# PABannier/bark.cpp

Measured on NVIDIA H100. Metric: audio sec/sec (inverse RTF), bark-small f16, batch 1 per GPU, semantic->coarse->fine->encodec, higher is better.
Workload: dtype f16 weights/operands, f32 accumulate (reference arithmetic)

## Files before the change

### bark.cpp_b200/__init__.py

```python
from __future__ import annotations

import ctypes as C
import os

import numpy as np

_HERE = os.path.dirname(os.path.abspath(__file__))
LIB_PATH = os.path.join(_HERE, "libbark_b200.so")

PROGRESS_CB = C.CFUNCTYPE(None, C.c_void_p, C.c_int, C.c_int, C.c_void_p)


class BarkContextParams(C.Structure):
    _fields_ = [
        ("verbosity", C.c_int), ("temp", C.c_float), ("fine_temp", C.c_float), ("min_eos_p", C.c_float),
        ("sliding_window_size", C.c_int32), ("max_coarse_history", C.c_int32), ("sample_rate", C.c_int32),
        ("target_bandwidth", C.c_int32), ("cls_token_id", C.c_int32), ("sep_token_id", C.c_int32),
        ("n_steps_text_encoder", C.c_int32), ("text_pad_token", C.c_int32), ("text_encoding_offset", C.c_int32),
        ("semantic_rate_hz", C.c_float), ("semantic_pad_token", C.c_int32), ("semantic_vocab_size", C.c_int32),
        ("semantic_infer_token", C.c_int32), ("coarse_rate_hz", C.c_float), ("coarse_infer_token", C.c_int32),
        ("coarse_semantic_pad_token", C.c_int32), ("n_coarse_codebooks", C.c_int32), ("n_fine_codebooks", C.c_int32),
        ("codebook_size", C.c_int32), ("progress_callback", PROGRESS_CB), ("progress_callback_user_data", C.c_void_p),
    ]


class BarkStatistics(C.Structure):
    _fields_ = [("t_load_us", C.c_int64), ("t_eval_us", C.c_int64), ("t_semantic_us", C.c_int64), ("t_coarse_us", C.c_int64),
                ("t_fine_us", C.c_int64), ("n_sample_semantic", C.c_int32), ("n_sample_coarse", C.c_int32), ("n_sample_fine", C.c_int32)]


EXPORTS = [
    "bark_context_default_params", "bark_load_model", "bark_generate_audio", "bark_get_audio_data", "bark_get_audio_data_size",
    "bark_get_load_time", "bark_get_eval_time", "bark_reset_statistics", "bark_model_quantize", "bark_free",
    "bark_b200_set_device", "bark_b200_version", "bark_b200_gpt_eval", "bark_b200_fine_eval", "bark_b200_encodec_decode",
    "bark_b200_sample", "bark_b200_sample_rows", "bark_b200_reseed", "bark_b200_tokenize", "bark_b200_forward_text_encoder",
    "bark_b200_forward_coarse_encoder", "bark_b200_forward_fine_encoder", "bark_b200_get_tokens", "bark_b200_set_tokens",
    "bark_b200_get_stats", "bark_b200_get_hparams", "bark_b200_kernel_launches", "bark_b200_layernorm_fallbacks",
    "bark_b200_profile_enable", "bark_b200_profile_report", "bark_b200_io_counters", "bark_b200_decode_timing",
    "bark_b200_shard_init", "bark_b200_shard_connect", "bark_b200_shard_nvlink_bytes",
    "bark_b200_fast_mode", "bark_b200_fast_gemm", "bark_b200_fast_attention",
    "bark_b200_generate_batch", "bark_b200_batch_audio", "bark_b200_batch_tokens", "bark_b200_gpt_eval_slot", "bark_b200_gpt_step_batch",
    "ggml_time_init", "ggml_time_us", "ggml_time_ms", "ggml_init", "ggml_free",
]

_lib = None


def lib() -> C.CDLL:
    global _lib
    if _lib is not None:
        return _lib
    if not os.path.exists(LIB_PATH):
        raise RuntimeError(f"{LIB_PATH} is missing: build the CUDA extension first (python -c 'import __graft_entry__ as g; g.build()'). "
                           "There is no CPU fallback.")
    L = C.CDLL(LIB_PATH)
    vp, i32p, f32p = C.c_void_p, C.c_void_p, C.c_void_p
    L.bark_context_default_params.restype = BarkContextParams
    L.bark_load_model.restype = vp
    L.bark_load_model.argtypes = [C.c_char_p, BarkContextParams, C.c_uint32]
    L.bark_generate_audio.restype = C.c_bool
    L.bark_generate_audio.argtypes = [vp, C.c_char_p, C.c_int]
    L.bark_get_audio_data.restype = C.POINTER(C.c_float)
    L.bark_get_audio_data.argtypes = [vp]
    L.bark_get_audio_data_size.restype = C.c_int
    L.bark_get_audio_data_size.argtypes = [vp]
    for n in ("bark_get_load_time", "bark_get_eval_time"):
        getattr(L, n).restype = C.c_int64
        getattr(L, n).argtypes = [vp]
    L.bark_reset_statistics.argtypes = [vp]
    L.bark_model_quantize.restype = C.c_bool
    L.bark_model_quantize.argtypes = [C.c_char_p, C.c_char_p, C.c_int]
    L.bark_free.argtypes = [vp]
    L.bark_b200_set_device.argtypes = [C.c_int]
    L.bark_b200_version.restype = C.c_char_p
    L.bark_b200_gpt_eval.restype = C.c_int
    L.bark_b200_gpt_eval.argtypes = [vp, C.c_int, i32p, C.c_int, C.POINTER(C.c_int), C.c_int, f32p]
    L.bark_b200_fine_eval.restype = C.c_int
    L.bark_b200_fine_eval.argtypes = [vp, i32p, C.c_int, f32p]
    L.bark_b200_encodec_decode.restype = C.c_int
    L.bark_b200_encodec_decode.argtypes = [vp, i32p, C.c_int, f32p, C.c_int]
    L.bark_b200_sample.restype = C.c_int
    L.bark_b200_sample.argtypes = [vp, C.c_int, f32p, C.c_int, C.c_float, C.POINTER(C.c_float)]
    L.bark_b200_sample_rows.restype = C.c_int
    L.bark_b200_sample_rows.argtypes = [vp, f32p, C.c_int, C.c_int, C.c_float, i32p, f32p]
    L.bark_b200_reseed.argtypes = [vp, C.c_uint32]
    L.bark_b200_tokenize.argtypes = [vp, C.c_char_p, i32p]
    for n in ("bark_b200_forward_text_encoder", "bark_b200_forward_coarse_encoder", "bark_b200_forward_fine_encoder"):
        getattr(L, n).restype = C.c_bool
        getattr(L, n).argtypes = [vp, C.c_int]
    L.bark_b200_get_tokens.restype = C.c_int
    L.bark_b200_get_tokens.argtypes = [vp, C.c_int, i32p, C.c_int]
    L.bark_b200_set_tokens.argtypes = [vp, C.c_int, i32p, C.c_int]
    L.bark_b200_get_stats.argtypes = [vp, C.POINTER(BarkStatistics), C.c_void_p]
    L.bark_b200_get_hparams.argtypes = [vp, C.c_int, i32p]
    L.bark_b200_kernel_launches.restype = C.c_ulonglong
    L.bark_b200_layernorm_fallbacks.restype = C.c_uint
    L.bark_b200_layernorm_fallbacks.argtypes = [vp]
    L.bark_b200_profile_enable.argtypes = [C.c_int]
    L.bark_b200_profile_report.restype = C.c_int
    L.bark_b200_profile_report.argtypes = [C.c_char_p, C.c_int]
    L.bark_b200_io_counters.argtypes = [C.POINTER(C.c_ulonglong), C.POINTER(C.c_ulonglong), C.c_int]
    L.bark_b200_decode_timing.restype = C.c_int
    L.bark_b200_decode_timing.argtypes = [vp, C.c_void_p, C.c_int]
    L.bark_b200_shard_init.restype = C.c_int
    L.bark_b200_shard_init.argtypes = [vp, C.c_int, C.c_int, vp]
    L.bark_b200_shard_connect.restype = C.c_int
    L.bark_b200_shard_connect.argtypes = [vp, vp]
    L.bark_b200_shard_nvlink_bytes.restype = C.c_ulonglong
    L.bark_b200_shard_nvlink_bytes.argtypes = [vp, C.c_int]
    L.bark_b200_fast_mode.restype = C.c_int
    L.bark_b200_fast_mode.argtypes = [vp]
    L.bark_b200_fast_gemm.restype = C.c_int
    L.bark_b200_fast_gemm.argtypes = [vp, vp, vp, C.c_int, C.c_int, C.c_int, C.c_int, C.c_int]
    L.bark_b200_fast_attention.restype = C.c_int
    L.bark_b200_fast_attention.argtypes = [vp, vp, vp, vp, C.c_int, C.c_int, C.c_int]
    L.bark_b200_generate_batch.restype = C.c_bool
    L.bark_b200_generate_batch.argtypes = [vp, C.POINTER(C.c_char_p), C.POINTER(C.c_uint32), C.c_int, C.c_int]
    L.bark_b200_batch_audio.restype = C.c_int
    L.bark_b200_batch_audio.argtypes = [vp, C.c_int, f32p, C.c_int]
    L.bark_b200_batch_tokens.restype = C.c_int
    L.bark_b200_batch_tokens.argtypes = [vp, C.c_int, C.c_int, i32p, C.c_int]
    L.bark_b200_gpt_eval_slot.restype = C.c_int
    L.bark_b200_gpt_eval_slot.argtypes = [vp, C.c_int, C.c_int, i32p, C.c_int, C.POINTER(C.c_int), C.c_int, f32p]
    L.bark_b200_gpt_step_batch.restype = C.c_int
    L.bark_b200_gpt_step_batch.argtypes = [vp, C.c_int, C.c_int, i32p, i32p, i32p, f32p]
    L.ggml_time_us.restype = C.c_int64
    _lib = L
    return L


def _p(a: np.ndarray):
    return a.ctypes.data_as(C.c_void_p)


class Bark:

    def __init__(self, model_path: str, seed: int = 0, n_steps_text_encoder: int | None = None, temp=None, fine_temp=None,
                 min_eos_p=None, device: int | None = None, progress=None):
        L = lib()
        p = L.bark_context_default_params()
        if n_steps_text_encoder is not None:
            p.n_steps_text_encoder = n_steps_text_encoder
        if temp is not None:
            p.temp = temp
        if fine_temp is not None:
            p.fine_temp = fine_temp
        if min_eos_p is not None:
            p.min_eos_p = min_eos_p
        self._cb = PROGRESS_CB(progress) if progress else PROGRESS_CB()
        p.progress_callback = self._cb
        if device is not None:
            L.bark_b200_set_device(device)
        self.params = p
        self.ctx = L.bark_load_model(os.fsencode(model_path), p, seed)
        if not self.ctx:
            raise RuntimeError(f"bark_load_model failed for {model_path} (see stderr); no CPU fallback exists")
        self.ctx = C.c_void_p(self.ctx)

    def close(self):
        if getattr(self, "ctx", None):
            lib().bark_free(self.ctx)
            self.ctx = None

    def __enter__(self):
        return self

    def __exit__(self, *a):
        self.close()

    def generate(self, text: str, n_threads: int = 1) -> np.ndarray:
        if not lib().bark_generate_audio(self.ctx, text.encode(), n_threads):
            raise RuntimeError("bark_generate_audio failed")
        n = lib().bark_get_audio_data_size(self.ctx)
        return np.ctypeslib.as_array(lib().bark_get_audio_data(self.ctx), shape=(n,)).copy()

    @property
    def load_time_us(self):
        return lib().bark_get_load_time(self.ctx)

    @property
    def eval_time_us(self):
        return lib().bark_get_eval_time(self.ctx)

    def hparams(self, which: int) -> np.ndarray:
        a = np.zeros(10, np.int32)
        lib().bark_b200_get_hparams(self.ctx, which, _p(a))
        return a

    def tokens(self, stage: int) -> np.ndarray:
        n = lib().bark_b200_get_tokens(self.ctx, stage, None, 0)
        a = np.zeros(max(n, 1), np.int32)
        lib().bark_b200_get_tokens(self.ctx, stage, _p(a), n)
        a = a[:n]
        return a.reshape(-1, 2) if stage == 1 else a.reshape(-1, 8) if stage == 2 else a

    def set_tokens(self, stage: int, arr):
        a = np.ascontiguousarray(arr, np.int32).ravel()
        lib().bark_b200_set_tokens(self.ctx, stage, _p(a), a.size)

    def tokenize(self, text: str) -> np.ndarray:
        a = np.zeros(513, np.int32)
        lib().bark_b200_tokenize(self.ctx, text.encode(), _p(a))
        return a

    def gpt_eval(self, which: int, tokens, n_past: int, merge_ctx: bool):
        t = np.ascontiguousarray(tokens, np.int32)
        out = np.zeros(int(self.hparams(which)[6]), np.float32)
        np_ = C.c_int(n_past)
        if not lib().bark_b200_gpt_eval(self.ctx, which, _p(t), t.size, C.byref(np_), int(merge_ctx), _p(out)):
            raise RuntimeError("bark_b200_gpt_eval failed")
        return out, np_.value

    def gpt_eval_slot(self, which: int, slot: int, tokens, n_past: int, merge_ctx: bool):
        t = np.ascontiguousarray(tokens, np.int32)
        out = np.zeros(int(self.hparams(which)[6]), np.float32)
        np_ = C.c_int(n_past)
        if not lib().bark_b200_gpt_eval_slot(self.ctx, which, slot, _p(t), t.size, C.byref(np_), int(merge_ctx), _p(out)):
            raise RuntimeError("bark_b200_gpt_eval_slot failed")
        return out, np_.value

    def gpt_step_batch(self, which: int, slots, tokens, n_past):
        sl = np.ascontiguousarray(slots, np.int32); t = np.ascontiguousarray(tokens, np.int32)
        npa = np.array(n_past, np.int32, copy=True)
        assert sl.size == t.size == npa.size
        out = np.zeros((sl.size, int(self.hparams(which)[6])), np.float32)
        if not lib().bark_b200_gpt_step_batch(self.ctx, which, sl.size, _p(sl), _p(t), _p(npa), _p(out)):
            raise RuntimeError("bark_b200_gpt_step_batch failed")
        return out, npa

    def generate_batch(self, texts, seeds, n_threads: int = 1) -> list:
        n = len(texts)
        if len(seeds) != n:
            raise RuntimeError(f"generate_batch: {n} prompts but {len(seeds)} seeds")
        arr = (C.c_char_p * max(n, 1))(*[t.encode() for t in texts])
        sd = (C.c_uint32 * max(n, 1))(*[int(s) for s in seeds])
        if not lib().bark_b200_generate_batch(self.ctx, arr, sd, n, n_threads):
            raise RuntimeError("bark_b200_generate_batch failed")
        out = []
        for i in range(n):
            m = lib().bark_b200_batch_audio(self.ctx, i, None, 0)
            a = np.zeros(max(m, 1), np.float32)
            lib().bark_b200_batch_audio(self.ctx, i, _p(a), m)
            out.append(a[:m])
        return out

    def batch_tokens(self, i: int, stage: int) -> np.ndarray:
        n = lib().bark_b200_batch_tokens(self.ctx, i, stage, None, 0)
        if n < 0:
            raise IndexError(f"no batch item {i}")
        a = np.zeros(max(n, 1), np.int32)
        lib().bark_b200_batch_tokens(self.ctx, i, stage, _p(a), n)
        a = a[:n]
        return a.reshape(-1, 2) if stage == 1 else a.reshape(-1, 8) if stage == 2 else a

    def fine_eval(self, in_buffer, nn: int) -> np.ndarray:
        t = np.ascontiguousarray(in_buffer, np.int32)
        assert t.size == 8 * 1024
        out = np.zeros((1024, int(self.hparams(2)[6])), np.float32)
        if not lib().bark_b200_fine_eval(self.ctx, _p(t), nn, _p(out)):
            raise RuntimeError("bark_b200_fine_eval failed")
        return out

    def encodec_decode(self, codes_8xT) -> np.ndarray:
        c = np.ascontiguousarray(codes_8xT, np.int32)
        T = c.shape[1]
        out = np.zeros(320 * T, np.float32)
        n = lib().bark_b200_encodec_decode(self.ctx, _p(c), T, _p(out), out.size)
        if n < 0:
            raise RuntimeError("bark_b200_encodec_decode failed")
        return out[:n]

    def sample(self, which: int, logits, temp: float):
        l = np.ascontiguousarray(logits, np.float32)
        e = C.c_float(0)
        return lib().bark_b200_sample(self.ctx, which, _p(l), l.size, temp, C.byref(e)), e.value

    def sample_rows(self, logits_rows, temp: float):
        l = np.ascontiguousarray(logits_rows, np.float32)
        rows, n = l.shape
        tok = np.zeros(rows, np.int32); eos = np.zeros(rows, np.float32)
        r = lib().bark_b200_sample_rows(self.ctx, _p(l), n, rows, temp, _p(tok), _p(eos))
        if r < 0:
            raise RuntimeError("bark_b200_sample_rows failed")
        return tok, eos, r

    def reseed(self, seed: int):
        lib().bark_b200_reseed(self.ctx, seed)

    def forward(self, stage: int):
        f = [lib().bark_b200_forward_text_encoder, lib().bark_b200_forward_coarse_encoder, lib().bark_b200_forward_fine_encoder][stage]
        if not f(self.ctx, 1):
            raise RuntimeError("stage failed")

    def stats(self):
        s = BarkStatistics()
        pm = np.zeros(9, np.int64)
        lib().bark_b200_get_stats(self.ctx, C.byref(s), _p(pm))
        return s, pm.reshape(3, 3)

    def shard_init(self, rank: int, world: int) -> bytes:
        h = C.create_string_buffer(64)
        if not lib().bark_b200_shard_init(self.ctx, rank, world, C.cast(h, C.c_void_p)):
            raise RuntimeError("bark_b200_shard_init failed")
        return h.raw

    def shard_connect(self, all_handles: bytes):
        buf = C.create_string_buffer(all_handles, len(all_handles))
        if not lib().bark_b200_shard_connect(self.ctx, C.cast(buf, C.c_void_p)):
            raise RuntimeError("bark_b200_shard_connect failed")

    def shard_nvlink_bytes(self, reset: bool = False) -> int:
        return int(lib().bark_b200_shard_nvlink_bytes(self.ctx, int(reset)))

    @property
    def fast_mode(self) -> bool:
        return bool(lib().bark_b200_fast_mode(self.ctx))

    def layernorm_fallbacks(self) -> int:
        return int(lib().bark_b200_layernorm_fallbacks(self.ctx))


FAST_EPILOGUES = {"f32": 0, "resid": 1, "gelu16": 2, "qkv16": 4}


class GuardBandError(RuntimeError):
    """The GEMM stored outside its output."""


def fast_gemm(A: np.ndarray, W: np.ndarray, epilogue: str = "f32", bn: int = 0, resid: np.ndarray | None = None, return_bn: bool = False):
    A = np.ascontiguousarray(A, np.float16); W = np.ascontiguousarray(W, np.float16)
    M, K = A.shape; N = W.shape[0]
    assert W.shape[1] == K, (A.shape, W.shape)
    if epilogue == "resid":
        out = np.array(resid, np.float32, order="C", copy=True)
        assert out.shape == (M, N), out.shape
    elif epilogue == "qkv16":
        assert N % 6 == 0, N
        out = np.zeros(M * N, np.float16)
    else:
        out = np.zeros((M, N), np.float16 if epilogue == "gelu16" else np.float32)
    r = lib().bark_b200_fast_gemm(_p(A), _p(W), _p(out), M, N, K, FAST_EPILOGUES[epilogue], bn)
    if r == -1:
        raise GuardBandError(f"bark_b200_fast_gemm ({epilogue}, {M}x{N}x{K}, bn {bn}) wrote outside its output")
    if r <= 0:
        raise RuntimeError(f"bark_b200_fast_gemm ({epilogue}, {M}x{N}x{K}, bn {bn}) failed")
    if epilogue == "qkv16":
        out = (out[:M * 2 * N // 3].reshape(M, 2 * N // 3), out[M * 2 * N // 3:].reshape(N // 3, M))
    return (out, r) if return_bn else out


def fast_attention(q: np.ndarray, k: np.ndarray, v: np.ndarray, n_head: int) -> np.ndarray:
    q, k, v = (np.ascontiguousarray(a, np.float16) for a in (q, k, v))
    n, E = q.shape
    out = np.zeros((n, E), np.float16)
    if not lib().bark_b200_fast_attention(_p(q), _p(k), _p(v), _p(out), n, E, n_head):
        raise RuntimeError("bark_b200_fast_attention failed")
    return out


def kernel_launches() -> int:
    return int(lib().bark_b200_kernel_launches())


def profile_enable(on: bool):
    lib().bark_b200_profile_enable(int(on))


def profile_report() -> dict:
    import json
    n = lib().bark_b200_profile_report(None, 0)
    buf = C.create_string_buffer(n + 16)
    lib().bark_b200_profile_report(buf, n + 16)
    return json.loads(buf.value.decode())


def io_counters(reset: bool = False):
    a, b = C.c_ulonglong(0), C.c_ulonglong(0)
    lib().bark_b200_io_counters(C.byref(a), C.byref(b), int(reset))
    return a.value, b.value
```

### bark.cpp_b200/csrc/bark_api.cu

```cuda
#include "../../include/bark_b200.h"
#include "context.h"
#include "gpt_kernels.h"

#include <algorithm>
#include <cmath>
#include <cstring>

using namespace bark;

namespace {

thread_local int g_device_override = -1;
bool quiet() { static const bool q = [] { const char * e = getenv("BARK_B200_QUIET"); return e && *e && *e != '0'; }(); return q; }

inline bool is_alpha(unsigned char c) { return (c >= 'a' && c <= 'z') || (c >= 'A' && c <= 'Z'); }
inline bool is_digit(unsigned char c) { return c >= '0' && c <= '9'; }
inline bool is_punct(unsigned char c) { return c > 32 && c < 127 && !is_alpha(c) && !is_digit(c); }

char fold_accent(unsigned char second) {
    const unsigned cp = 0xC0u + (second - 0x80u);
    const bool lower = cp >= 0xE0;
    const unsigned up = lower ? cp - 0x20 : cp;
    char base = 0;
    if (up >= 0xC0 && up <= 0xC5) base = 'A';
    else if (up == 0xC7) base = 'C';
    else if (up >= 0xC8 && up <= 0xCB) base = 'E';
    else if (up >= 0xCC && up <= 0xCF) base = 'I';
    else if (up == 0xD1) base = 'N';
    else if (up >= 0xD2 && up <= 0xD6) base = 'O';
    else if (up >= 0xD9 && up <= 0xDC) base = 'U';
    else if (up == 0xDD) base = 'Y';
    if (!base) return 0;
    return lower ? (char)(base + 32) : base;
}

std::string strip_accents_utf8(const std::string & in) {
    std::string out;
    for (size_t i = 0; i < in.size();) {
        const unsigned char c = (unsigned char) in[i];
        const unsigned hi = c >> 4;
        size_t len = hi < 12 ? 1 : hi < 14 ? 2 : hi == 14 ? 3 : 4;
        len = std::min(len, in.size() - i);
        char folded = 0;
        if (len == 2 && c == 0xC3) { const unsigned char d = (unsigned char) in[i + 1]; if (d >= 0x80 && d <= 0xBF) folded = fold_accent(d); }
        if (folded) out.push_back(folded); else out.append(in, i, len);
        i += len;
    }
    return out;
}

void wordpiece(const std::map<std::string, int32_t> & vocab, const std::string & text, std::vector<int32_t> & out, int n_max_tokens) {
    const std::string s = strip_accents_utf8(text);
    out.clear();
    size_t i = 0;
    while (i < s.size()) {
        const unsigned char c = (unsigned char) s[i];
        size_t j = i;
        if (is_punct(c)) j = i + 1;
        else if (is_alpha(c)) { while (j < s.size() && is_alpha((unsigned char) s[j])) j++; }
        else if (is_digit(c)) { while (j < s.size() && is_digit((unsigned char) s[j])) j++; }
        else { i++; continue; }
        const std::string word = s.substr(i, j - i);
        i = j;
        size_t p = 0; bool cont = false;
        while (p < word.size()) {
            if ((int) out.size() >= n_max_tokens - 1) break;
            size_t e = word.size(); bool hit = false;
            for (; e > p; e--) {
                auto it = vocab.find((cont ? "##" : "") + word.substr(p, e - p));
                if (it != vocab.end()) { out.push_back(it->second); p = e; cont = true; hit = true; break; }
            }
            if (!hit) { fprintf(stderr, "%s: unknown token '%c'\n", "bert_tokenize", word[p]); cont = true; p++; }
        }
    }
}

void tokenize_input(bark_context * ctx, Generation & g, const std::string & text) {
    const bark_context_params & P = ctx->params;
    const int max_ctx = std::min(ctx->semantic.block_size, 256);
    std::vector<int32_t> pieces;
    wordpiece(ctx->token_to_id, text, pieces, max_ctx);
    std::vector<int32_t> t((size_t) max_ctx, 0);
    std::copy(pieces.begin(), pieces.end(), t.begin());
    for (auto & v : t) v += P.text_encoding_offset;
    for (size_t k = pieces.size(); k < t.size(); k++) t[k] = P.text_pad_token;
    t.insert(t.end(), 256, P.semantic_pad_token);
    t.push_back(P.semantic_infer_token);
    g.tokens = t;
    if (!quiet()) {
        printf("%s: prompt: '%s'\n", "bark_tokenize_input", text.c_str());
        printf("%s: number of tokens in prompt = %zu, first 8 tokens: ", "bark_tokenize_input", g.tokens.size());
        for (size_t k = 0; k < std::min<size_t>(8, g.tokens.size()); k++) printf("%d ", g.tokens[k]);
        printf("\n\n");
    }
}

int32_t sample_token(std::mt19937 & rng, GPTModel & m, const float * logits, int n, float temp, float * eos_p) {
    const int64_t t0 = now_us();
    std::vector<float> p(logits, logits + n);
    const float div = temp == 0.0f ? 0.7f : temp;
    for (float & v : p) v /= div;
    float mx = -INFINITY;
    for (float v : p) mx = std::max(mx, v);
    float sum = 0.0f;
    for (float & v : p) { v = (float) exp((double)(v - mx)); sum += v; }
    for (float & v : p) v /= sum;
    int32_t next = 0;
    if (temp == 0.0f) {
        float best = -INFINITY;
        for (int i = 0; i < n; i++) if (p[(size_t) i] > best) { best = p[(size_t) i]; next = i; }
    } else {
        std::discrete_distribution<int32_t> dist(p.begin(), p.end());
        next = dist(rng);
    }
    if (eos_p) *eos_p = p.back();
    m.t_sample_us += now_us() - t0;
    m.n_sample += 1;
    return next;
}

}

int32_t bark::sample_token_given_u(const float * logits, int n, float temp, double u, float * eos_p) {
    std::vector<float> p(logits, logits + n);
    const float div = temp == 0.0f ? 0.7f : temp;
    for (float & v : p) v /= div;
    float mx = -INFINITY;
    for (float v : p) mx = std::max(mx, v);
    float sum = 0.0f;
    for (float & v : p) { v = (float) exp((double)(v - mx)); sum += v; }
    for (float & v : p) v /= sum;
    if (eos_p) *eos_p = p.back();
    if (temp == 0.0f) {
        float best = -INFINITY; int32_t next = 0;
        for (int i = 0; i < n; i++) if (p[(size_t) i] > best) { best = p[(size_t) i]; next = i; }
        return next;
    }
    std::vector<double> cp(p.begin(), p.end());
    double tot = 0.0;
    for (double v : cp) tot += v;
    for (double & v : cp) v /= tot;
    for (size_t i = 1; i < cp.size(); i++) cp[i] += cp[i - 1];
    cp.back() = 1.0;
    return (int32_t)(std::lower_bound(cp.begin(), cp.end(), u) - cp.begin());
}

namespace {

void print_stage_stats(const GPTModel & m) {
    if (quiet()) return;
    printf("\n\n");
    printf("%s:   sample time = %8.2f ms / %lld tokens\n", "bark_print_statistics", m.t_sample_us / 1000.0f, (long long) m.n_sample);
    printf("%s:  predict time = %8.2f ms / %.2f ms per token\n", "bark_print_statistics", m.t_predict_us / 1000.0f,
           m.n_sample ? m.t_predict_us / (double) m.n_sample / 1000.0 : 0.0);
    printf("%s:    total time = %8.2f ms\n", "bark_print_statistics", m.t_main_us / 1000.0f);
    printf("\n");
}

template <typename LoOf>
bool run_chain(bark_context * ctx, std::mt19937 & rng, GPTModel & m, const std::vector<int32_t> & first_in, bool merge_ctx, int * n_past, int n, LoOf lo_of, int samp_n, float temp,
               int32_t * out_tok, float * out_eos) {
    if (n < 1 || n > 1024) return false;
    const int64_t t_begin = now_us();
    cudaStream_t s = ctx->stream;
    if (temp != 0.0f) {
        for (int j = 0; j < n; j++) ctx->h_u[j] = std::generate_canonical<double, 53>(rng);
        BARK_CUDA_CHECK(cudaMemcpyAsync(ctx->d_u, ctx->h_u, (size_t) n * sizeof(double), cudaMemcpyHostToDevice, s)); bark::g_h2d_bytes += (size_t) n * sizeof(double);
    }
    const bool chain = ctx->use_decode_kernel && m.decode_ok;
    std::vector<int> past_before((size_t) n);
    std::vector<int32_t> cur_in = first_in;
    std::vector<float> host_logits;
    int start = 0;
    while (start < n) {
        const int stop = chain ? n : start + 1;
        for (int j = start; j < stop; j++) {
            const int lo = lo_of(j);
            past_before[(size_t) j] = *n_past;
            if (j == start) { if (!gpt_eval(ctx, m, cur_in.data(), (int) cur_in.size(), n_past, merge_ctx && *n_past == 0, nullptr, lo, lo + samp_n)) return false; }
            const int force = ctx->debug_flag_every > 0 && (ctx->n_sample_calls++ % ctx->debug_flag_every) == 0;
            if (j > start && !gpt_decode_chained(ctx, m, ctx->d_feed, n_past, lo, lo + samp_n)) return false;
            sample_rows(ctx->last_logits + lo, m.n_out_vocab, samp_n, 1, temp, ctx->d_u + j, ctx->d_stok + j, lo, ctx->d_feed, ctx->d_seos + j, ctx->d_sflags + j, force, s);
        }
        const size_t cnt = (size_t)(stop - start);
        BARK_CUDA_CHECK(cudaMemcpyAsync(ctx->h_stok + start, ctx->d_stok + start, cnt * 4, cudaMemcpyDeviceToHost, s));
        BARK_CUDA_CHECK(cudaMemcpyAsync(ctx->h_sflags + start, ctx->d_sflags + start, cnt * 4, cudaMemcpyDeviceToHost, s));
        BARK_CUDA_CHECK(cudaMemcpyAsync(ctx->h_seos + start, ctx->d_seos + start, cnt * 4, cudaMemcpyDeviceToHost, s)); bark::g_d2h_bytes += cnt * 12;
        BARK_CUDA_CHECK(cudaStreamSynchronize(s));
        int f = start;
        while (f < stop && !ctx->h_sflags[f]) f++;
        if (f == stop) { start = stop; if (start < n) cur_in.assign(1, ctx->h_stok[start - 1]); continue; }
        if (f > start) cur_in.assign(1, ctx->h_stok[f - 1]);
        *n_past = past_before[(size_t) f];
        const int lo = lo_of(f);
        host_logits.resize((size_t) m.n_out_vocab);
        if (!gpt_eval(ctx, m, cur_in.data(), (int) cur_in.size(), n_past, merge_ctx && *n_past == 0, host_logits.data(), lo, lo + samp_n)) return false;
        ctx->h_stok[f] = lo + sample_token_given_u(host_logits.data() + lo, samp_n, temp, ctx->h_u[f], &ctx->h_seos[f]);
        ctx->n_sample_host_replays++;
        start = f + 1;
        cur_in.assign(1, ctx->h_stok[f]);
    }
    for (int j = 0; j < n; j++) { out_tok[j] = ctx->h_stok[j]; if (out_eos) out_eos[j] = ctx->h_seos[j]; }
    m.n_sample += n;
    m.t_predict_us += now_us() - t_begin;
    return true;
}

bool run_semantic(bark_context * ctx, Generation & g) {
    const int64_t t_start = now_us();
    GPTModel & m = ctx->semantic;
    const bark_context_params & P = ctx->params;
    std::vector<float> logits((size_t) m.n_out_vocab);
    std::vector<int32_t> input = g.tokens, output;
    int n_past = 0; float eos_p = 0.0f;
    const bool dev = ctx->sample_on_device && (size_t) m.n_out_vocab * 4 <= 64 * 1024;
    if (dev) {
        constexpr int kBatch = 64;
        std::vector<int32_t> tok(kBatch); std::vector<float> eos(kBatch);
        bool done = false;
        for (int i = 0; i < P.n_steps_text_encoder && !done; i += kBatch) {
            const int nb = std::min(kBatch, P.n_steps_text_encoder - i);
            const std::mt19937 saved = g.rng;
            if (!run_chain(ctx, g.rng, m, input, true, &n_past, nb, [](int) { return 0; }, m.n_out_vocab, P.temp, tok.data(), eos.data())) { fprintf(stderr, "%s: Could not generate token\n", __func__); return false; }
            for (int j = 0; j < nb; j++) {
                if (P.progress_callback) P.progress_callback(ctx, SEMANTIC, 100 * (i + j + 1) / P.n_steps_text_encoder, P.progress_callback_user_data);
                if (tok[(size_t) j] == P.semantic_vocab_size || eos[(size_t) j] >= P.min_eos_p) {
                    if (P.temp != 0.0f) { g.rng = saved; for (int k = 0; k <= j; k++) (void) std::generate_canonical<double, 53>(g.rng); }
                    m.n_sample -= nb - (j + 1);
                    done = true; break;
                }
                output.push_back(tok[(size_t) j]);
            }
            if (!done && nb > 0) input.assign(1, tok[(size_t) nb - 1]);
        }
    } else
    for (int i = 0; i < P.n_steps_text_encoder; i++) {
        if (P.progress_callback) P.progress_callback(ctx, SEMANTIC, 100 * (i + 1) / P.n_steps_text_encoder, P.progress_callback_user_data);
        if (!gpt_eval(ctx, m, input.data(), (int) input.size(), &n_past, true, logits.data())) { fprintf(stderr, "%s: Could not generate token\n", __func__); return false; }
        const int32_t next = sample_token(g.rng, m, logits.data(), m.n_out_vocab, P.temp, &eos_p);
        if (next == P.semantic_vocab_size || eos_p >= P.min_eos_p) break;
        input.assign(1, next);
        output.push_back(next);
    }
    g.semantic_tokens = output;
    ctx->stats.n_sample_semantic = (int32_t) m.n_sample;
    m.t_main_us = now_us() - t_start;
    ctx->stats.t_semantic_us = m.t_main_us;
    print_stage_stats(m);
    return true;
}

int coarse_n_steps(const bark_context_params & P, size_t n_semantic) {
    const float stc_ratio = P.coarse_rate_hz / P.semantic_rate_hz * P.n_coarse_codebooks;
    return (int)(floorf(n_semantic * stc_ratio / P.n_coarse_codebooks) * P.n_coarse_codebooks);
}

std::vector<int32_t> coarse_window(bark_context * ctx, const std::vector<int32_t> & sem, const std::vector<int32_t> & out, int step,
                                   std::vector<int32_t> & kv_ids, size_t & kv_canon, int * n_past) {
    const bark_context_params & P = ctx->params;
    const float stc_ratio = P.coarse_rate_hz / P.semantic_rate_hz * P.n_coarse_codebooks;
    const int max_semantic_history = (int) floorf(P.max_coarse_history / stc_ratio);
    const int semantic_idx = (int) roundf(step / stc_ratio);
    std::vector<int32_t> in(sem.begin() + std::max(semantic_idx - max_semantic_history, 0), sem.end());
    in.resize(256, P.coarse_semantic_pad_token);
    in.push_back(P.coarse_infer_token);
    const size_t hist = std::min<size_t>((size_t) P.max_coarse_history, out.size());
    in.insert(in.end(), out.end() - (std::ptrdiff_t) hist, out.end());
    *n_past = 0;
    if (ctx->kv_reuse) {
        size_t common = 0;
        while (common < kv_ids.size() && common < in.size() && kv_ids[common] == in[common]) common++;
        *n_past = (int) std::min({common, kv_canon, in.size() & ~(size_t) 31, in.size() - 1});
        ctx->n_kv_reused += (unsigned long long) *n_past;
    }
    kv_canon = std::max((size_t) *n_past, in.size() & ~(size_t) 31);
    std::vector<int32_t> in_eval(in.begin() + *n_past, in.end());
    kv_ids = in;
    return in_eval;
}

void store_coarse_tokens(const bark_context_params & P, const std::vector<int32_t> & out, std::vector<int32_t> & coarse) {
    coarse.resize(out.size());
    for (size_t i = 0; i + 1 < out.size(); i += 2) {
        coarse[i] = out[i] - P.semantic_vocab_size;
        coarse[i + 1] = out[i + 1] - P.semantic_vocab_size - P.codebook_size;
    }
}

bool run_coarse(bark_context * ctx, Generation & g) {
    const int64_t t_start = now_us();
    GPTModel & m = ctx->coarse;
    const bark_context_params & P = ctx->params;
    const std::vector<int32_t> & sem = g.semantic_tokens;
    std::vector<float> logits((size_t) m.n_out_vocab);
    const int n_steps = coarse_n_steps(P, sem.size());
    if (n_steps <= 0 || P.n_coarse_codebooks != 2) { fprintf(stderr, "%s: nothing to generate (%zu semantic tokens)\n", __func__, sem.size()); return false; }
    const int n_windows = (int) ceilf((float) n_steps / P.sliding_window_size);
    std::vector<int32_t> out; out.reserve((size_t) n_steps);
    const bool dev = ctx->sample_on_device && P.sliding_window_size <= 1024 && P.semantic_vocab_size + 2 * P.codebook_size <= m.n_out_vocab;
    int step = 0;
    std::vector<int32_t> kv_ids;
    size_t kv_canon = 0;
    for (int w = 0; w < n_windows; w++) {
        int n_past = 0;
        std::vector<int32_t> in_eval = coarse_window(ctx, sem, out, step, kv_ids, kv_canon, &n_past);
        if (dev) {
            const int nw = std::min(P.sliding_window_size, n_steps - step), step0 = step;
            std::vector<int32_t> tok((size_t) nw);
            auto lo_of = [&](int j) { return P.semantic_vocab_size + (((step0 + j) % P.n_coarse_codebooks == 0) ? 0 : 1) * P.codebook_size; };
            if (!run_chain(ctx, g.rng, m, in_eval, false, &n_past, nw, lo_of, P.codebook_size, P.temp, tok.data(), nullptr)) { fprintf(stderr, "%s: Could not generate token\n", __func__); return false; }
            for (int j = 0; j < nw; j++) {
                if (P.progress_callback) P.progress_callback(ctx, COARSE, 100 * (step + 1) / n_steps, P.progress_callback_user_data);
                out.push_back(tok[(size_t) j]); step++;
                if (j + 1 < nw) kv_ids.push_back(tok[(size_t) j]);
            }
            continue;
        }
        for (int j = 0; j < P.sliding_window_size && step < n_steps; j++) {
            if (P.progress_callback) P.progress_callback(ctx, COARSE, 100 * (step + 1) / n_steps, P.progress_callback_user_data);
            const bool major = step % P.n_coarse_codebooks == 0;
            const int lo = P.semantic_vocab_size + (major ? 0 : 1) * P.codebook_size;
            if (j > 0) kv_ids.push_back(in_eval[0]);
            if (!gpt_eval(ctx, m, in_eval.data(), (int) in_eval.size(), &n_past, false, logits.data(), lo, lo + P.codebook_size)) { fprintf(stderr, "%s: Could not generate token\n", __func__); return false; }
            const int32_t next = lo + sample_token(g.rng, m, logits.data() + lo, P.codebook_size, P.temp, nullptr);
            in_eval.assign(1, next);
            out.push_back(next);
            step++;
        }
    }
    store_coarse_tokens(P, out, g.coarse_tokens);
    ctx->stats.n_sample_coarse = (int32_t) m.n_sample;
    m.t_main_us = now_us() - t_start;
    ctx->stats.t_coarse_us = m.t_main_us;
    print_stage_stats(m);
    return true;
}

bool run_fine(bark_context * ctx, Generation & g, bool progress = true) {
    const int64_t t_start = now_us();
    GPTModel & m = ctx->fine;
    const bark_context_params & P = ctx->params;
    const int n_coarse = P.n_coarse_codebooks, n_cb = P.n_fine_codebooks, cb_size = P.codebook_size;
    if (n_cb != 8 || n_coarse != 2 || cb_size != 1024) { fprintf(stderr, "%s: unsupported codebook configuration\n", __func__); return false; }
    const int T = (int) g.coarse_tokens.size() / 2;
    const int len = std::max(T, 1024);
    std::vector<int32_t> arr((size_t) len * 8, cb_size);
    for (int t = 0; t < T; t++) { arr[(size_t) t * 8] = g.coarse_tokens[(size_t) t * 2]; arr[(size_t) t * 8 + 1] = g.coarse_tokens[(size_t) t * 2 + 1]; }
    const int n_loops = std::max(0, (int) ceilf((len - 1024) / 512.f)) + 1;
    std::vector<float> logits((size_t) 1024 * m.n_out_vocab);
    std::vector<int32_t> buf((size_t) 8 * 1024), sampled(1024);
    const bool dev = ctx->sample_on_device;
    for (int n = 0; n < n_loops; n++) {
        const int start = std::min(n * 512, len - 1024), fill = std::min(n * 512, len - 512), rel = fill - start;
        for (int c = 0; c < 8; c++) for (int j = 0; j < 1024; j++) buf[(size_t) c * 1024 + j] = arr[(size_t)(start + j) * 8 + c];
        for (int nn = n_coarse; nn < n_cb; nn++) {
            if (progress && P.progress_callback) P.progress_callback(ctx, FINE, 100 * (n * (n_cb - n_coarse) + (nn - n_coarse + 1)) / (n_loops * (n_cb - n_coarse)), P.progress_callback_user_data);
            if (ctx->shard.on) {
                if (!fine_eval_shard(ctx, buf.data(), nn) || !sample_shard(ctx, g.rng, cb_size, P.fine_temp, sampled.data())) { fprintf(stderr, "%s: Could not generate token\n", __func__); return false; }
            } else {
            if (!fine_eval(ctx, buf.data(), nn, dev ? nullptr : logits.data())) { fprintf(stderr, "%s: Could not generate token\n", __func__); return false; }
            if (dev && !sample_device(ctx, m, g.rng, ctx->last_logits, m.n_out_vocab, cb_size, 1024, P.fine_temp, sampled.data(), nullptr)) return false;
            }
            for (int i = 0; i < 1024; i++) {
                const int32_t next = (dev || ctx->shard.on) ? sampled[(size_t) i] : sample_token(g.rng, m, logits.data() + (size_t) i * m.n_out_vocab, cb_size, P.fine_temp, nullptr);
                if (i >= rel) buf[(size_t) nn * 1024 + i] = next;
            }
        }
        for (int nn = n_coarse; nn < n_cb; nn++) for (int j = 0; j < 1024 - rel; j++) arr[(size_t)(fill + j) * 8 + nn] = buf[(size_t) nn * 1024 + rel + j];
    }
    g.fine_tokens.assign(arr.begin(), arr.begin() + (std::ptrdiff_t) T * 8);
    ctx->stats.n_sample_fine = (int32_t) m.n_sample;
    m.t_main_us = now_us() - t_start;
    ctx->stats.t_fine_us = m.t_main_us;
    print_stage_stats(m);
    return true;
}

bool decode_audio(bark_context * ctx, Generation & g) {
    const int T = (int) g.fine_tokens.size() / 8;
    std::vector<int32_t> codes((size_t) 8 * T);
    for (int c = 0; c < 8; c++) for (int t = 0; t < T; t++) codes[(size_t) c * T + t] = g.fine_tokens[(size_t) t * 8 + c];
    if (ctx->params.target_bandwidth != 6 || ctx->params.sample_rate != 24000) {
        fprintf(stderr, "%s: only target_bandwidth 6 / 24 kHz is implemented\n", __func__); return false;
    }
    if (!codec_decode(ctx, codes.data(), T, g.audio)) { printf("%s: Could not generate waveform from tokens with Encodec\n", __func__); return false; }
    return true;
}

constexpr int kMaxBatch = 8;

bool ensure_batch_slots(bark_context * ctx, int n) {
    BatchSlots & S = ctx->batch;
    auto fail = [&](const char * what) { (void) cudaGetLastError(); fprintf(stderr, "bark_b200: out of device memory for %s\n", what); return false; };
    if (!S.d_logits) {
        const size_t n_out = (size_t) std::max(ctx->semantic.n_out_vocab, ctx->coarse.n_out_vocab);
        float * l = nullptr; int32_t * d = nullptr, * h = nullptr;
        if (cudaMalloc(&l, kMaxBatch * n_out * 4) != cudaSuccess) return fail("the batch logits");
        if (cudaMalloc(&d, 16 * 4) != cudaSuccess) { cudaFree(l); return fail("the batch logits"); }
        if (cudaMallocHost(&h, 16 * 4) != cudaSuccess) { cudaFree(l); cudaFree(d); return fail("the batch logits"); }
        S.d_logits = l; S.d_step = d; S.h_step = h;
    }
    for (; S.cap < n; S.cap++) {
        float * slab[4] = {nullptr, nullptr, nullptr, nullptr};
        size_t bytes[4];
        for (int j = 0; j < 4; j++) {
            const GPTModel & m = j < 2 ? ctx->semantic : ctx->coarse;
            bytes[j] = (size_t) m.n_layer * m.block_size * m.n_embd * 4;
            if (cudaMalloc(&slab[j], bytes[j]) != cudaSuccess) {
                for (int q = 0; q < j; q++) cudaFree(slab[q]);
                return fail("a batch item's KV cache");
            }
        }
        for (int j = 0; j < 4; j++) BARK_CUDA_CHECK(cudaMemsetAsync(slab[j], 0, bytes[j], ctx->stream));
        S.k[0][S.cap] = slab[0]; S.v[0][S.cap] = slab[1]; S.k[1][S.cap] = slab[2]; S.v[1][S.cap] = slab[3];
    }
    return true;
}

struct BatchItem {
    Generation g;
    int n_past = 0;
    std::vector<int32_t> out, kv_ids;
    size_t kv_canon = 0;
    int n_steps = 0;
};

bool batch_prefill(bark_context * ctx, GPTModel & m, int which, BatchItem & it, int b, int row, const std::vector<int32_t> & in, bool merge, int lo, int hi) {
    BatchSlots & S = ctx->batch;
    if (!gpt_eval(ctx, m, in.data(), (int) in.size(), &it.n_past, merge, nullptr, lo, hi, S.k[which][b], S.v[which][b])) return false;
    BARK_CUDA_CHECK(cudaMemcpyAsync(S.d_logits + (size_t) row * m.n_out_vocab, ctx->last_logits, (size_t) m.n_out_vocab * 4, cudaMemcpyDeviceToDevice, ctx->stream));
    BARK_CUDA_CHECK(cudaStreamSynchronize(ctx->stream));
    return true;
}

bool batch_sample(bark_context * ctx, GPTModel & m, std::vector<BatchItem> & items, const std::vector<int> & act, int lo, int n, float temp, int32_t * tok, float * eos) {
    const int64_t t0 = now_us();
    cudaStream_t s = ctx->stream;
    const int B = (int) act.size();
    if ((size_t) n * 4 > 64 * 1024) { fprintf(stderr, "%s: %d logits per row exceed the device sampler's row\n", __func__, n); return false; }
    if (temp != 0.0f) {
        for (int r = 0; r < B; r++) ctx->h_u[r] = std::generate_canonical<double, 53>(items[(size_t) act[(size_t) r]].g.rng);
        BARK_CUDA_CHECK(cudaMemcpyAsync(ctx->d_u, ctx->h_u, (size_t) B * sizeof(double), cudaMemcpyHostToDevice, s)); g_h2d_bytes += (size_t) B * sizeof(double);
    }
    const int force = ctx->debug_flag_every > 0 && (ctx->n_sample_calls++ % ctx->debug_flag_every) == 0;
    const float * logits = ctx->batch.d_logits;
    sample_rows(logits + lo, m.n_out_vocab, n, B, temp, ctx->d_u, ctx->d_stok, lo, nullptr, ctx->d_seos, ctx->d_sflags, force, s);
    BARK_CUDA_CHECK(cudaMemcpyAsync(ctx->h_stok, ctx->d_stok, (size_t) B * 4, cudaMemcpyDeviceToHost, s));
    BARK_CUDA_CHECK(cudaMemcpyAsync(ctx->h_sflags, ctx->d_sflags, (size_t) B * 4, cudaMemcpyDeviceToHost, s));
    BARK_CUDA_CHECK(cudaMemcpyAsync(ctx->h_seos, ctx->d_seos, (size_t) B * 4, cudaMemcpyDeviceToHost, s)); g_d2h_bytes += (size_t) B * 12;
    BARK_CUDA_CHECK(cudaStreamSynchronize(s));
    std::vector<float> row;
    for (int r = 0; r < B; r++) {
        if (ctx->h_sflags[r]) {
            row.resize((size_t) n);
            BARK_CUDA_CHECK(cudaMemcpy(row.data(), logits + (size_t) r * m.n_out_vocab + lo, (size_t) n * 4, cudaMemcpyDeviceToHost)); g_d2h_bytes += (size_t) n * 4;
            ctx->h_stok[r] = lo + sample_token_given_u(row.data(), n, temp, ctx->h_u[r], &ctx->h_seos[r]);
            ctx->n_sample_host_replays++;
        }
        tok[r] = ctx->h_stok[r]; eos[r] = ctx->h_seos[r];
    }
    m.n_sample += B;
    m.t_sample_us += now_us() - t0;
    return true;
}

bool batch_step(bark_context * ctx, GPTModel & m, int which, std::vector<BatchItem> & items, const std::vector<int> & act, const int32_t * tok, int lo, int hi) {
    float * sk[kMaxBatch], * sv[kMaxBatch]; int pos[kMaxBatch];
    for (size_t r = 0; r < act.size(); r++) { sk[r] = ctx->batch.k[which][act[r]]; sv[r] = ctx->batch.v[which][act[r]]; pos[r] = items[(size_t) act[r]].n_past; }
    if (!gpt_step_batch(ctx, m, (int) act.size(), sk, sv, tok, pos, lo, hi, ctx->batch.d_logits)) return false;
    for (int b : act) items[(size_t) b].n_past++;
    return true;
}

bool batch_semantic(bark_context * ctx, std::vector<BatchItem> & items) {
    GPTModel & m = ctx->semantic;
    const bark_context_params & P = ctx->params;
    std::vector<int> act;
    for (int b = 0; b < (int) items.size() && P.n_steps_text_encoder > 0; b++) {
        items[(size_t) b].n_past = 0;
        if (!batch_prefill(ctx, m, 0, items[(size_t) b], b, b, items[(size_t) b].g.tokens, true, 0, 0)) return false;
        act.push_back(b);
    }
    int32_t tok[kMaxBatch]; float eos[kMaxBatch];
    while (!act.empty()) {
        if (!batch_sample(ctx, m, items, act, 0, m.n_out_vocab, P.temp, tok, eos)) return false;
        std::vector<int> next; int32_t next_tok[kMaxBatch];
        for (size_t r = 0; r < act.size(); r++) {
            Generation & g = items[(size_t) act[r]].g;
            if (tok[r] == P.semantic_vocab_size || eos[r] >= P.min_eos_p) continue;
            g.semantic_tokens.push_back(tok[r]);
            if ((int) g.semantic_tokens.size() < P.n_steps_text_encoder) { next_tok[next.size()] = tok[r]; next.push_back(act[r]); }
        }
        act.swap(next);
        if (!act.empty() && !batch_step(ctx, m, 0, items, act, next_tok, 0, 0)) return false;
    }
    return true;
}

bool batch_coarse(bark_context * ctx, std::vector<BatchItem> & items) {
    GPTModel & m = ctx->coarse;
    const bark_context_params & P = ctx->params;
    if (P.n_coarse_codebooks != 2 || P.semantic_vocab_size + 2 * P.codebook_size > m.n_out_vocab) { fprintf(stderr, "%s: unsupported codebook configuration\n", __func__); return false; }
    int n_windows = 0;
    for (BatchItem & it : items) {
        it.n_steps = coarse_n_steps(P, it.g.semantic_tokens.size());
        if (it.n_steps <= 0) { fprintf(stderr, "%s: nothing to generate (%zu semantic tokens)\n", __func__, it.g.semantic_tokens.size()); return false; }
        n_windows = std::max(n_windows, (int) ceilf((float) it.n_steps / P.sliding_window_size));
        it.out.clear(); it.kv_ids.clear(); it.kv_canon = 0;
    }
    auto lo_of = [&](int step) { return P.semantic_vocab_size + ((step % P.n_coarse_codebooks == 0) ? 0 : 1) * P.codebook_size; };
    int32_t tok[kMaxBatch]; float eos[kMaxBatch];
    for (int w = 0; w < n_windows; w++) {
        const int step0 = w * P.sliding_window_size, lo0 = lo_of(step0);
        std::vector<int> act;
        for (int b = 0; b < (int) items.size(); b++) {
            BatchItem & it = items[(size_t) b];
            if (step0 >= it.n_steps) continue;
            const std::vector<int32_t> in_eval = coarse_window(ctx, it.g.semantic_tokens, it.out, step0, it.kv_ids, it.kv_canon, &it.n_past);
            if (!batch_prefill(ctx, m, 1, it, b, (int) act.size(), in_eval, false, lo0, lo0 + P.codebook_size)) return false;
            act.push_back(b);
        }
        for (int j = 0; !act.empty(); j++) {
            const int lo = lo_of(step0 + j);
            if (!batch_sample(ctx, m, items, act, lo, P.codebook_size, P.temp, tok, eos)) return false;
            std::vector<int> next; int32_t next_tok[kMaxBatch];
            for (size_t r = 0; r < act.size(); r++) {
                BatchItem & it = items[(size_t) act[r]];
                it.out.push_back(tok[r]);
                if (j + 1 < std::min(P.sliding_window_size, it.n_steps - step0)) {
                    it.kv_ids.push_back(tok[r]);
                    next_tok[next.size()] = tok[r]; next.push_back(act[r]);
                }
            }
            act.swap(next);
            const int lo_next = lo_of(step0 + j + 1);
            if (!act.empty() && !batch_step(ctx, m, 1, items, act, next_tok, lo_next, lo_next + P.codebook_size)) return false;
        }
    }
    for (BatchItem & it : items) store_coarse_tokens(P, it.out, it.g.coarse_tokens);
    return true;
}

struct BatchGuard {
    bark_context * ctx; bark_statistics stats; int64_t counters[3][4]; bool keep_stats = false;
    GPTModel * model(int i) const { return i == 0 ? &ctx->semantic : i == 1 ? &ctx->coarse : &ctx->fine; }
    explicit BatchGuard(bark_context * c) : ctx(c), stats(c->stats) {
        for (int i = 0; i < 3; i++) { const GPTModel & m = *model(i); counters[i][0] = m.n_sample; counters[i][1] = m.t_sample_us; counters[i][2] = m.t_predict_us; counters[i][3] = m.t_main_us; }
    }
    int32_t samples(int i) const { return (int32_t)(model(i)->n_sample - counters[i][0]); }
    ~BatchGuard() {
        for (int i = 0; i < 3; i++) { GPTModel & m = *model(i); m.n_sample = counters[i][0]; m.t_sample_us = counters[i][1]; m.t_predict_us = counters[i][2]; m.t_main_us = counters[i][3]; }
        if (!keep_stats) ctx->stats = stats;
    }
};

bool generate_batch(bark_context * ctx, const char * const * texts, const uint32_t * seeds, int n) {
    if (!ctx) { fprintf(stderr, "%s: invalid bark context\n", __func__); return false; }
    if (n < 1 || n > kMaxBatch) { fprintf(stderr, "%s: %d prompts (1 to %d per batch)\n", __func__, n, kMaxBatch); return false; }
    if (!texts || !seeds) { fprintf(stderr, "%s: null prompts or seeds\n", __func__); return false; }
    for (int i = 0; i < n; i++) if (!texts[i]) { fprintf(stderr, "%s: prompt %d is null\n", __func__, i); return false; }
    if (ctx->shard.on) { fprintf(stderr, "%s: not available on a context whose fine stage is sharded over GPUs\n", __func__); return false; }
    BARK_CUDA_CHECK(cudaSetDevice(ctx->device));
    if (!ensure_batch_slots(ctx, n)) return false;
    BatchGuard guard(ctx);
    bark_statistics st{};
    st.t_load_us = ctx->stats.t_load_us;
    const int64_t t0 = now_us();
    std::vector<BatchItem> items((size_t) n);
    for (int i = 0; i < n; i++) { items[(size_t) i].g.rng = std::mt19937(seeds[i]); tokenize_input(ctx, items[(size_t) i].g, texts[i]); }
    bool ok = batch_semantic(ctx, items);
    const int64_t t1 = now_us();
    ok = ok && batch_coarse(ctx, items);
    const int64_t t2 = now_us();
    st.n_sample_semantic = guard.samples(0);
    st.n_sample_coarse = guard.samples(1);
    int64_t t_fine = 0;
    for (int i = 0; ok && i < n; i++) {
        const int64_t tf = now_us();
        ok = run_fine(ctx, items[(size_t) i].g, false);
        t_fine += now_us() - tf;
        ok = ok && decode_audio(ctx, items[(size_t) i].g);
    }
    st.n_sample_fine = guard.samples(2);
    if (!ok) return false;
    st.t_semantic_us = t1 - t0; st.t_coarse_us = t2 - t1; st.t_fine_us = t_fine; st.t_eval_us = now_us() - t0;
    ctx->stats = st; guard.keep_stats = true;
    ctx->batch.results.clear();
    for (BatchItem & it : items) ctx->batch.results.push_back(std::move(it.g));
    return true;
}

void alloc_workspace(bark_context * ctx) {
    int E = 0, H = 0; size_t kp_bytes = 0, n_logits = 0;
    for (GPTModel * m : {&ctx->semantic, &ctx->coarse, &ctx->fine}) {
        E = std::max(E, (int) m->n_embd); H = std::max(H, (int) m->n_head);
        const size_t es = m->wtype == W_F16 ? 2 : 4;
        kp_bytes = std::max(kp_bytes, (size_t) li_padded_k(4 * m->n_embd, (int) es) * es);
    }
    n_logits = std::max<size_t>({(size_t) ctx->semantic.n_out_vocab, (size_t) ctx->coarse.n_out_vocab, (size_t) 1024 * ctx->fine.n_out_vocab});
    Workspace & ws = ctx->ws;
    const size_t R = 1024;
    ws.max_rows = (int) R; ws.E = E;
    ws.x    = (float *) ctx_alloc(ctx, R * E * 4);
    ws.act  = ctx_alloc(ctx, R * kp_bytes);
    ws.act2 = ctx_alloc(ctx, R * kp_bytes);
    ws.q    = (float *) ctx_alloc(ctx, R * E * 4);
    ws.kbuf = (float *) ctx_alloc(ctx, R * E * 4);
    ws.vbuf = (float *) ctx_alloc(ctx, R * E * 4);
    ws.scores = (float *) ctx_alloc(ctx, (size_t) H * R * R * 4);
    ws.logits = (float *) ctx_alloc(ctx, n_logits * 4);
    ws.tok  = (int32_t *) ctx_alloc(ctx, 8 * 1024 * 4);
    if (is_quant(ctx->semantic.wtype) || is_quant(ctx->coarse.wtype) || is_quant(ctx->fine.wtype)) {
        ctx->d_q8 = ctx_alloc(ctx, R * (size_t) 4 * E); ctx->d_q8_scales = ctx_alloc(ctx, R * (size_t)(4 * E / 32) * 4);
        ctx->d_q8_sums = ctx_alloc(ctx, R * (size_t)(4 * E / 32) * 4);
    }
    if (ctx->fast_mode) {
        const GPTModel & fm = ctx->fine;
        if (fm.wtype != W_F16 || fm.n_embd / fm.n_head != 64 || fm.n_embd % 64 != 0 || fm.n_embd > 1024) {
            fprintf(stderr, "bark_b200: BARK_B200_MODE=fast needs f16 fine-model weights with 64-wide heads; using the parity path\n");
            ctx->fast_mode = false;
        } else {
            const size_t FE = (size_t) fm.n_embd;
            ctx->f_a16 = (__half *) ctx_alloc(ctx, R * FE * 2); ctx->f_h16 = (__half *) ctx_alloc(ctx, R * 4 * FE * 2);
            ctx->f_qk16 = (__half *) ctx_alloc(ctx, R * 2 * FE * 2); ctx->f_vt16 = (__half *) ctx_alloc(ctx, FE * R * 2); ctx->f_att16 = (__half *) ctx_alloc(ctx, R * FE * 2);
        }
    }
    BARK_CUDA_CHECK(cudaMallocHost(&ctx->h_logits, n_logits * 4));
    BARK_CUDA_CHECK(cudaMallocHost(&ctx->h_tok, 8 * 1024 * 4));
    ctx->d_u = (double *) ctx_alloc(ctx, 1024 * 8); ctx->d_stok = (int32_t *) ctx_alloc(ctx, 1024 * 4);
    ctx->d_sflags = (int32_t *) ctx_alloc(ctx, 1024 * 4); ctx->d_seos = (float *) ctx_alloc(ctx, 1024 * 4);
    ctx->d_feed = (int32_t *) ctx_alloc(ctx, 64); BARK_CUDA_CHECK(cudaMemset(ctx->d_feed, 0, 64));
    BARK_CUDA_CHECK(cudaMemset(ctx->d_u, 0, 1024 * 8));
    BARK_CUDA_CHECK(cudaMallocHost(&ctx->h_u, 1024 * 8)); BARK_CUDA_CHECK(cudaMallocHost(&ctx->h_stok, 1024 * 4));
    BARK_CUDA_CHECK(cudaMallocHost(&ctx->h_sflags, 1024 * 4)); BARK_CUDA_CHECK(cudaMallocHost(&ctx->h_seos, 1024 * 4));
}

}

extern "C" struct ggml_context * ggml_init(struct ggml_init_params) { static int token; return reinterpret_cast<struct ggml_context *>(&token); }
extern "C" void    ggml_free(struct ggml_context *) {}
extern "C" void    ggml_time_init(void) {}
extern "C" int64_t ggml_time_us(void) { return now_us(); }
extern "C" int64_t ggml_time_ms(void) { return now_us() / 1000; }

extern "C" struct bark_context_params bark_context_default_params(void) {
    bark_context_params p;
    memset(&p, 0, sizeof(p));
    p.verbosity = LOW;
    p.temp = 0.7f; p.fine_temp = 0.5f; p.min_eos_p = 0.2f;
    p.sliding_window_size = 60; p.max_coarse_history = 630;
    p.sample_rate = 24000; p.target_bandwidth = 6;
    p.cls_token_id = 101; p.sep_token_id = 102;
    p.n_steps_text_encoder = 768;
    p.text_pad_token = 129595; p.text_encoding_offset = 10048;
    p.semantic_rate_hz = 49.9f; p.semantic_pad_token = 10000; p.semantic_vocab_size = 10000; p.semantic_infer_token = 129599;
    p.coarse_rate_hz = 75.0f; p.coarse_infer_token = 12050; p.coarse_semantic_pad_token = 12048;
    p.n_coarse_codebooks = 2; p.n_fine_codebooks = 8; p.codebook_size = 1024;
    p.progress_callback = nullptr; p.progress_callback_user_data = nullptr;
    return p;
}

extern "C" void bark_b200_set_device(int device) { g_device_override = device; }

extern "C" struct bark_context * bark_load_model(const char * model_path, struct bark_context_params params, uint32_t seed) {
    const int64_t t0 = now_us();
    if (!model_path) { fprintf(stderr, "%s: null model path\n", __func__); return nullptr; }
    int n_dev = 0;
    if (cudaGetDeviceCount(&n_dev) != cudaSuccess || n_dev == 0) {
        fprintf(stderr, "%s: no CUDA device available — this library has no CPU path\n", __func__);
        return nullptr;
    }
    int dev = g_device_override;
    if (dev < 0) { const char * e = getenv("BARK_B200_DEVICE"); dev = e ? atoi(e) : 0; }
    if (dev < 0 || dev >= n_dev) { fprintf(stderr, "%s: CUDA device %d out of range (%d present)\n", __func__, dev, n_dev); return nullptr; }
    cudaDeviceProp prop;
    if (cudaSetDevice(dev) != cudaSuccess || cudaGetDeviceProperties(&prop, dev) != cudaSuccess) { fprintf(stderr, "%s: cannot use CUDA device %d: %s\n", __func__, dev, cudaGetErrorString(cudaGetLastError())); return nullptr; }
    if (prop.major != 9 || prop.minor != 0) {
        fprintf(stderr, "%s: device %d is sm_%d%d; this library is built for sm_90a (H100) only\n", __func__, dev, prop.major, prop.minor);
        return nullptr;
    }
    bark_context * ctx = new bark_context();
    ctx->device = dev;
    ctx->n_sm = ctx->n_sm_total = prop.multiProcessorCount;
    if (ctx->n_sm >= 132) ctx->n_sm = 128;
    { const char * e = getenv("BARK_B200_MODE"); ctx->fast_mode = e && !strcmp(e, "fast"); }
    { const char * e = getenv("BARK_B200_DECODE_CTAS"); if (e && atoi(e) >= 64 && atoi(e) <= ctx->n_sm) ctx->n_sm = atoi(e); }
    { const char * e = getenv("BARK_B200_SAMPLE_FLAG_EVERY"); ctx->debug_flag_every = e ? atoi(e) : 0; }
    { const char * e = getenv("BARK_B200_SAMPLE"); ctx->sample_on_device = !(e && !strcmp(e, "host")); }
    { const char * e = getenv("BARK_B200_KV_REUSE"); ctx->kv_reuse = !(e && !strcmp(e, "0")); }
    { const char * e = getenv("BARK_B200_DECODE"); ctx->use_decode_kernel = !(e && !strcmp(e, "multi")); ctx->decode_cluster = e && !strcmp(e, "cluster"); }
    { const char * e = getenv("BARK_B200_DECODE_TIMING_TID"); if (e && atoi(e) >= 0 && atoi(e) < 512) ctx->timing_tid = atoi(e) & ~31; }
    { const char * e = getenv("BARK_B200_POLL_NS"); if (e && atoi(e) >= 0 && atoi(e) <= 100000) ctx->poll_ns = (unsigned) atoi(e); }
    { const char * e = getenv("BARK_B200_HEADSTART"); if (e) { unsigned v[6]; if (sscanf(e, "%u:%u:%u:%u:%u:%u", &v[0], &v[1], &v[2], &v[3], &v[4], &v[5]) == 6) for (int i = 0; i < 6; i++) ctx->headstart[i] = std::min(v[i], 100000u); } }
    ctx->params = params;
    const bool loaded = guarded(false, [&] {
    BARK_CUDA_CHECK(cudaStreamCreateWithFlags(&ctx->stream, cudaStreamNonBlocking));
    if (!load_model_file(model_path, ctx)) return false;
    alloc_workspace(ctx);
    { const char * e = getenv("BARK_B200_TAG_BASE"); if (e) ctx->tag_base = (unsigned) strtoul(e, nullptr, 0); }
    if (getenv("BARK_B200_DECODE_TIMING")) { ctx->d_timing = (unsigned long long *) ctx_alloc(ctx, 256 * 32 * 8); BARK_CUDA_CHECK(cudaMemset(ctx->d_timing, 0, 256 * 32 * 8)); }
    BARK_CUDA_CHECK(cudaStreamSynchronize(ctx->stream));
    return true;
    });
    if (!loaded) {
        fprintf(stderr, "%s: failed to load model weights from '%s'\n", __func__, model_path);
        bark_free(ctx);
        return nullptr;
    }
    ctx->gen.rng = std::mt19937(seed);
    ctx->stats.t_load_us = now_us() - t0;
    return ctx;
}

extern "C" void bark_reset_statistics(struct bark_context * ctx) {
    if (!ctx) return;
    const int64_t load = ctx->stats.t_load_us;
    memset(&ctx->stats, 0, sizeof(ctx->stats));
    ctx->stats.t_load_us = load;
}

extern "C" bool bark_b200_forward_text_encoder(struct bark_context * ctx, int) { return guarded(false, [&] { return ctx && run_semantic(ctx, ctx->gen); }); }
extern "C" bool bark_b200_forward_coarse_encoder(struct bark_context * ctx, int) { return guarded(false, [&] { return ctx && run_coarse(ctx, ctx->gen); }); }
extern "C" bool bark_b200_forward_fine_encoder(struct bark_context * ctx, int) { return guarded(false, [&] { return ctx && run_fine(ctx, ctx->gen); }); }
BARK_API bool bark_forward_text_encoder(struct bark_context * ctx, int n) { return bark_b200_forward_text_encoder(ctx, n); }
BARK_API bool bark_forward_coarse_encoder(struct bark_context * ctx, int n) { return bark_b200_forward_coarse_encoder(ctx, n); }
BARK_API bool bark_forward_fine_encoder(struct bark_context * ctx, int n) { return bark_b200_forward_fine_encoder(ctx, n); }

static bool bark_generate_audio_impl(struct bark_context * ctx, const char * text, int n_threads) {
    (void) n_threads;
    if (!ctx) { fprintf(stderr, "%s: invalid bark context\n", __func__); return false; }
    if (!text) { fprintf(stderr, "%s: null prompt\n", __func__); return false; }
    bark_reset_statistics(ctx);
    const int64_t t0 = now_us();
    BARK_CUDA_CHECK(cudaSetDevice(ctx->device));
    Generation & g = ctx->gen;
    tokenize_input(ctx, g, text);
    if (!run_semantic(ctx, g)) { fprintf(stderr, "%s: failed to forward text encoder\n", __func__); return false; }
    if (!run_coarse(ctx, g))   { fprintf(stderr, "%s: failed to forward coarse encoder\n", __func__); return false; }
    if (!run_fine(ctx, g))     { fprintf(stderr, "%s: failed to forward fine encoder\n", __func__); return false; }
    if (!decode_audio(ctx, g)) return false;
    ctx->stats.t_eval_us = now_us() - t0;
    return true;
}
extern "C" bool bark_generate_audio(struct bark_context * ctx, const char * text, int n_threads) { return guarded((bool) false, [&] { return bark_generate_audio_impl(ctx, text, n_threads); }); }

extern "C" float * bark_get_audio_data(struct bark_context * ctx) {
    if (!ctx) { fprintf(stderr, "%s: invalid bark context\n", __func__); return nullptr; }
    return ctx->gen.audio.empty() ? nullptr : ctx->gen.audio.data();
}
extern "C" int bark_get_audio_data_size(struct bark_context * ctx) {
    if (!ctx) { fprintf(stderr, "%s: invalid bark context\n", __func__); return 0; }
    return (int) ctx->gen.audio.size();
}
extern "C" int64_t bark_get_load_time(struct bark_context * ctx) {
    if (!ctx) { fprintf(stderr, "%s: invalid bark context\n", __func__); return 0; }
    return ctx->stats.t_load_us;
}
extern "C" int64_t bark_get_eval_time(struct bark_context * ctx) {
    if (!ctx) { fprintf(stderr, "%s: invalid bark context\n", __func__); return 0; }
    return ctx->stats.t_eval_us;
}

extern "C" void bark_free(struct bark_context * ctx) {
    if (!ctx) return;
    cudaSetDevice(ctx->device);
    if (ctx->stream) cudaStreamSynchronize(ctx->stream);
    for (void * p : ctx->device_allocs) cudaFree(p);
    for (int p = 0; p < ctx->shard.world; p++) if (p != ctx->shard.rank && ctx->shard.peer[p]) cudaIpcCloseMemHandle(ctx->shard.peer[p]);
    if (ctx->shard.local) cudaFree(ctx->shard.local);
    for (int i = 0; i < 3; i++) if (ctx->c_buf[i]) cudaFree(ctx->c_buf[i]);
    if (ctx->c_gi) cudaFree(ctx->c_gi);
    if (ctx->d_codes) cudaFree(ctx->d_codes);
    if (ctx->h_logits) cudaFreeHost(ctx->h_logits);
    if (ctx->h_tok) cudaFreeHost(ctx->h_tok);
    if (ctx->h_u) cudaFreeHost(ctx->h_u);
    if (ctx->h_stok) cudaFreeHost(ctx->h_stok);
    if (ctx->h_sflags) cudaFreeHost(ctx->h_sflags);
    if (ctx->h_seos) cudaFreeHost(ctx->h_seos);
    for (int w = 0; w < 2; w++) for (int b = 0; b < ctx->batch.cap; b++) { cudaFree(ctx->batch.k[w][b]); cudaFree(ctx->batch.v[w][b]); }
    if (ctx->batch.d_logits) cudaFree(ctx->batch.d_logits);
    if (ctx->batch.d_step) cudaFree(ctx->batch.d_step);
    if (ctx->batch.h_step) cudaFreeHost(ctx->batch.h_step);
    if (ctx->stream) cudaStreamDestroy(ctx->stream);
    delete ctx;
}

static GPTModel * pick(bark_context * ctx, int which) { return which == 0 ? &ctx->semantic : which == 1 ? &ctx->coarse : which == 2 ? &ctx->fine : nullptr; }

static int bark_b200_gpt_eval_impl(struct bark_context * ctx, int which, const int32_t * tokens, int n, int * n_past, int merge_ctx, float * logits_out) {
    if (!ctx || which < 0 || which > 1 || !tokens || !logits_out) return 0;
    BARK_CUDA_CHECK(cudaSetDevice(ctx->device));
    return gpt_eval(ctx, *pick(ctx, which), tokens, n, n_past, merge_ctx != 0, logits_out) ? 1 : 0;
}
extern "C" int bark_b200_gpt_eval(struct bark_context * ctx, int which, const int32_t * tokens, int n, int * n_past, int merge_ctx, float * logits_out) { return guarded((int) 0, [&] { return bark_b200_gpt_eval_impl(ctx, which, tokens, n, n_past, merge_ctx, logits_out); }); }
static int bark_b200_fine_eval_impl(struct bark_context * ctx, const int32_t * in_buffer, int nn, float * logits_out) {
    if (!ctx || !in_buffer || !logits_out) return 0;
    BARK_CUDA_CHECK(cudaSetDevice(ctx->device));
    return fine_eval(ctx, in_buffer, nn, logits_out) ? 1 : 0;
}
extern "C" int bark_b200_fine_eval(struct bark_context * ctx, const int32_t * in_buffer, int nn, float * logits_out) { return guarded((int) 0, [&] { return bark_b200_fine_eval_impl(ctx, in_buffer, nn, logits_out); }); }
static int bark_b200_encodec_decode_impl(struct bark_context * ctx, const int32_t * codes, int n_frames, float * out, int out_cap) {
    if (!ctx || !codes) return -1;
    BARK_CUDA_CHECK(cudaSetDevice(ctx->device));
    if (!codec_decode(ctx, codes, n_frames, ctx->gen.audio)) return -1;
    const int n = (int) ctx->gen.audio.size();
    if (out) memcpy(out, ctx->gen.audio.data(), sizeof(float) * (size_t) std::min(n, out_cap));
    return n;
}
extern "C" int bark_b200_encodec_decode(struct bark_context * ctx, const int32_t * codes, int n_frames, float * out, int out_cap) { return guarded((int) -1, [&] { return bark_b200_encodec_decode_impl(ctx, codes, n_frames, out, out_cap); }); }
extern "C" int bark_b200_sample(struct bark_context * ctx, int which, const float * logits, int n, float temp, float * eos_p) {
    if (!ctx || !logits || n < 1) return -1;
    return sample_token(ctx->gen.rng, *pick(ctx, which < 0 || which > 2 ? 0 : which), logits, n, temp, eos_p);
}
static int bark_b200_sample_rows_impl(struct bark_context * ctx, const float * logits, int n, int rows, float temp, int32_t * tokens_out, float * eos_p_out) {
    if (!ctx || !logits || !tokens_out || rows < 1 || rows > 1024 || n < 2 || (size_t) n * 4 > 64 * 1024) return -1;
    const size_t cap = std::max<size_t>({(size_t) ctx->semantic.n_out_vocab, (size_t) ctx->coarse.n_out_vocab, (size_t) 1024 * ctx->fine.n_out_vocab});
    if ((size_t) rows * n > cap) return -1;
    BARK_CUDA_CHECK(cudaSetDevice(ctx->device));
    BARK_CUDA_CHECK(cudaMemcpyAsync(ctx->ws.logits, logits, (size_t) rows * n * 4, cudaMemcpyHostToDevice, ctx->stream));
    const long long before = ctx->n_sample_host_replays;
    if (!sample_device(ctx, ctx->fine, ctx->gen.rng, ctx->ws.logits, n, n, rows, temp, tokens_out, eos_p_out)) return -1;
    return (int)(ctx->n_sample_host_replays - before);
}
extern "C" int bark_b200_sample_rows(struct bark_context * ctx, const float * logits, int n, int rows, float temp, int32_t * tokens_out, float * eos_p_out) { return guarded((int) -1, [&] { return bark_b200_sample_rows_impl(ctx, logits, n, rows, temp, tokens_out, eos_p_out); }); }
extern "C" void bark_b200_reseed(struct bark_context * ctx, uint32_t seed) { if (ctx) ctx->gen.rng = std::mt19937(seed); }
extern "C" void bark_b200_tokenize(struct bark_context * ctx, const char * text, int32_t * out513) {
    if (!ctx || !text || !out513) return;
    tokenize_input(ctx, ctx->gen, text);
    memcpy(out513, ctx->gen.tokens.data(), sizeof(int32_t) * 513);
}
static int copy_tokens(const Generation & g, int stage, int32_t * out, int cap) {
    const std::vector<int32_t> * v = stage == 0 ? &g.semantic_tokens : stage == 1 ? &g.coarse_tokens : stage == 2 ? &g.fine_tokens : stage == 3 ? &g.tokens : nullptr;
    if (!v) return -1;
    if (out) memcpy(out, v->data(), sizeof(int32_t) * std::min(v->size(), (size_t) std::max(cap, 0)));
    return (int) v->size();
}
extern "C" int bark_b200_get_tokens(struct bark_context * ctx, int stage, int32_t * out, int cap) { return ctx ? copy_tokens(ctx->gen, stage, out, cap) : -1; }
extern "C" void bark_b200_set_tokens(struct bark_context * ctx, int stage, const int32_t * in, int n) {
    if (!ctx || !in || n < 0) return;
    Generation & g = ctx->gen;
    if (stage == 0) g.semantic_tokens.assign(in, in + n); else if (stage == 1) g.coarse_tokens.assign(in, in + n); else if (stage == 3) g.tokens.assign(in, in + n);
}
extern "C" void bark_b200_get_stats(struct bark_context * ctx, struct bark_statistics * out, int64_t * per_model9) {
    if (!ctx) return;
    if (out) *out = ctx->stats;
    if (per_model9) { const GPTModel * m[3] = {&ctx->semantic, &ctx->coarse, &ctx->fine}; for (int i = 0; i < 3; i++) { per_model9[3 * i] = m[i]->t_predict_us; per_model9[3 * i + 1] = m[i]->t_sample_us; per_model9[3 * i + 2] = m[i]->n_sample; } }
}
extern "C" void bark_b200_get_hparams(struct bark_context * ctx, int which, int32_t * out10) {
    if (!ctx || !out10) return;
    const GPTModel * m = pick(ctx, which); if (!m) return;
    const int32_t v[10] = {m->n_layer, m->n_head, m->n_embd, m->block_size, m->bias, m->n_in_vocab, m->n_out_vocab, m->n_lm_heads, m->n_wtes, m->ftype};
    memcpy(out10, v, sizeof(v));
}
extern "C" unsigned long long bark_b200_kernel_launches(void) { return g_kernel_launches.load(); }
static unsigned bark_b200_layernorm_fallbacks_impl(struct bark_context * ctx) {
    if (!ctx) return 0;
    unsigned v = 0; BARK_CUDA_CHECK(cudaMemcpy(&v, ctx->d_ln_fallbacks, sizeof(v), cudaMemcpyDeviceToHost)); return v;
}
extern "C" unsigned bark_b200_layernorm_fallbacks(struct bark_context * ctx) { return guarded((unsigned) 0, [&] { return bark_b200_layernorm_fallbacks_impl(ctx); }); }
static int bark_b200_decode_timing_impl(struct bark_context * ctx, unsigned long long * out, int n) {
    if (!ctx || !ctx->d_timing || !out) return 0;
    BARK_CUDA_CHECK(cudaMemcpy(out, ctx->d_timing, sizeof(unsigned long long) * (size_t) std::min(n, 256 * 32), cudaMemcpyDeviceToHost));
    return std::min(n, 256 * 32);
}
extern "C" int bark_b200_decode_timing(struct bark_context * ctx, unsigned long long * out, int n) { return guarded((int) 0, [&] { return bark_b200_decode_timing_impl(ctx, out, n); }); }
static int bark_b200_fast_gemm_impl(const uint16_t * A, const uint16_t * W, void * C, int M, int N, int K, int epilogue, int bn) {
    if (!A || !W || !C || M < 1 || N < 1 || K < 64 || K % 64) return 0;
    if (epilogue != FEPI_F32 && epilogue != FEPI_RESID && epilogue != FEPI_GELU16 && epilogue != FEPI_QKV16) return 0;
    if (epilogue == FEPI_QKV16 && N % 6) return 0;
    constexpr size_t kGuard = 4096;
    constexpr unsigned char kPattern = 0x5a;
    size_t bytes[2] = {(size_t) M * N * (epilogue == FEPI_GELU16 ? 2 : 4), 0};
    if (epilogue == FEPI_QKV16) { bytes[0] = (size_t) M * (2 * N / 3) * 2; bytes[1] = (size_t) M * (N / 3) * 2; }
    __half * dA, * dW; unsigned char * reg[2] = {nullptr, nullptr}; int dev = 0, n_sm = 0;
    BARK_CUDA_CHECK(cudaGetDevice(&dev)); BARK_CUDA_CHECK(cudaDeviceGetAttribute(&n_sm, cudaDevAttrMultiProcessorCount, dev));
    BARK_CUDA_CHECK(cudaMalloc(&dA, (size_t) M * K * 2)); BARK_CUDA_CHECK(cudaMalloc(&dW, (size_t) N * K * 2));
    BARK_CUDA_CHECK(cudaMemcpy(dA, A, (size_t) M * K * 2, cudaMemcpyHostToDevice)); BARK_CUDA_CHECK(cudaMemcpy(dW, W, (size_t) N * K * 2, cudaMemcpyHostToDevice));
    for (int r = 0; r < 2 && bytes[r]; r++) {
        BARK_CUDA_CHECK(cudaMalloc(&reg[r], bytes[r] + 2 * kGuard));
        BARK_CUDA_CHECK(cudaMemset(reg[r], kPattern, bytes[r] + 2 * kGuard));
        if (epilogue == FEPI_RESID) BARK_CUDA_CHECK(cudaMemcpy(reg[r] + kGuard, C, bytes[r], cudaMemcpyHostToDevice));
        else                        BARK_CUDA_CHECK(cudaMemset(reg[r] + kGuard, 0xff, bytes[r]));
    }
    FastEpi ep; ep.mode = epilogue; ep.ldo = N;
    if (epilogue == FEPI_F32 || epilogue == FEPI_RESID) ep.out32 = (float *)(reg[0] + kGuard);
    else                                                ep.out16 = (__half *)(reg[0] + kGuard);
    if (epilogue == FEPI_QKV16) { ep.ldo = 2 * N / 3; ep.vt = (__half *)(reg[1] + kGuard); ep.vt_ld = M; ep.v_col0 = 2 * N / 3; }
    const int ran = fast_gemm(dA, K, dW, K, M, N, K, ep, n_sm, bn, 0);
    const cudaError_t e = cudaDeviceSynchronize();
    bool guards_intact = true;
    if (e != cudaSuccess) fprintf(stderr, "bark_b200_fast_gemm: %s\n", cudaGetErrorString(e));
    else {
        std::vector<unsigned char> g(kGuard);
        size_t off = 0;
        for (int r = 0; r < 2 && bytes[r]; r++) {
            for (const unsigned char * band : {reg[r], reg[r] + kGuard + bytes[r]}) {
                BARK_CUDA_CHECK(cudaMemcpy(g.data(), band, kGuard, cudaMemcpyDeviceToHost));
                for (unsigned char b : g) guards_intact &= b == kPattern;
            }
            BARK_CUDA_CHECK(cudaMemcpy((unsigned char *) C + off, reg[r] + kGuard, bytes[r], cudaMemcpyDeviceToHost));
            off += bytes[r];
        }
    }
    cudaFree(dA); cudaFree(dW); cudaFree(reg[0]); cudaFree(reg[1]);
    if (!ran || e != cudaSuccess) return 0;
    if (!guards_intact) { fprintf(stderr, "bark_b200_fast_gemm: a store landed outside the output (guard band overwritten)\n"); return -1; }
    return ran;
}
extern "C" int bark_b200_fast_gemm(const uint16_t * A, const uint16_t * W, void * C, int M, int N, int K, int epilogue, int bn) {
    return guarded((int) 0, [&] { return bark_b200_fast_gemm_impl(A, W, C, M, N, K, epilogue, bn); });
}
static int bark_b200_fast_attention_impl(const uint16_t * q, const uint16_t * k, const uint16_t * v, uint16_t * out, int n, int E, int H) {
    if (!q || !k || !v || !out || n < 128 || n % 128 || E != H * 64) return 0;
    std::vector<uint16_t> qk((size_t) n * 2 * E), vt((size_t) E * n);
    for (int r = 0; r < n; r++) {
        memcpy(&qk[(size_t) r * 2 * E], q + (size_t) r * E, (size_t) E * 2); memcpy(&qk[(size_t) r * 2 * E + E], k + (size_t) r * E, (size_t) E * 2);
        for (int c = 0; c < E; c++) vt[(size_t) c * n + r] = v[(size_t) r * E + c];
    }
    __half * dqk, * dvt, * dout;
    BARK_CUDA_CHECK(cudaMalloc(&dqk, qk.size() * 2)); BARK_CUDA_CHECK(cudaMalloc(&dvt, vt.size() * 2)); BARK_CUDA_CHECK(cudaMalloc(&dout, (size_t) n * E * 2));
    BARK_CUDA_CHECK(cudaMemcpy(dqk, qk.data(), qk.size() * 2, cudaMemcpyHostToDevice)); BARK_CUDA_CHECK(cudaMemcpy(dvt, vt.data(), vt.size() * 2, cudaMemcpyHostToDevice));
    const bool ok = fast_attention(dqk, 2 * E, E, dvt, n, E, H, dout, 0);
    const cudaError_t e = cudaDeviceSynchronize();
    if (e != cudaSuccess) fprintf(stderr, "bark_b200_fast_attention: %s\n", cudaGetErrorString(e));
    else BARK_CUDA_CHECK(cudaMemcpy(out, dout, (size_t) n * E * 2, cudaMemcpyDeviceToHost));
    cudaFree(dqk); cudaFree(dvt); cudaFree(dout);
    return ok && e == cudaSuccess;
}
extern "C" int bark_b200_fast_attention(const uint16_t * q, const uint16_t * k, const uint16_t * v, uint16_t * out, int n, int E, int H) { return guarded((int) 0, [&] { return bark_b200_fast_attention_impl(q, k, v, out, n, E, H); }); }
extern "C" int bark_b200_fast_mode(struct bark_context * ctx) { return ctx && ctx->fast_mode ? 1 : 0; }

extern "C" bool bark_b200_generate_batch(struct bark_context * ctx, const char * const * texts, const uint32_t * seeds, int n, int n_threads) {
    (void) n_threads;
    return guarded(false, [&] { return generate_batch(ctx, texts, seeds, n); });
}
extern "C" int bark_b200_batch_audio(struct bark_context * ctx, int i, float * out, int cap) {
    if (!ctx || i < 0 || i >= (int) ctx->batch.results.size()) return -1;
    const std::vector<float> & a = ctx->batch.results[(size_t) i].audio;
    if (out) memcpy(out, a.data(), sizeof(float) * std::min(a.size(), (size_t) std::max(cap, 0)));
    return (int) a.size();
}
extern "C" int bark_b200_batch_tokens(struct bark_context * ctx, int i, int stage, int32_t * out, int cap) {
    if (!ctx || i < 0 || i >= (int) ctx->batch.results.size()) return -1;
    return copy_tokens(ctx->batch.results[(size_t) i], stage, out, cap);
}
static int bark_b200_gpt_eval_slot_impl(struct bark_context * ctx, int which, int slot, const int32_t * tokens, int n, int * n_past, int merge_ctx, float * logits_out) {
    if (!ctx || which < 0 || which > 1 || slot < 0 || slot >= kMaxBatch || !tokens || !n_past || !logits_out) return 0;
    BARK_CUDA_CHECK(cudaSetDevice(ctx->device));
    if (!ensure_batch_slots(ctx, slot + 1)) return 0;
    return gpt_eval(ctx, *pick(ctx, which), tokens, n, n_past, merge_ctx != 0, logits_out, 0, 0, ctx->batch.k[which][slot], ctx->batch.v[which][slot]) ? 1 : 0;
}
extern "C" int bark_b200_gpt_eval_slot(struct bark_context * ctx, int which, int slot, const int32_t * tokens, int n, int * n_past, int merge_ctx, float * logits_out) {
    return guarded((int) 0, [&] { return bark_b200_gpt_eval_slot_impl(ctx, which, slot, tokens, n, n_past, merge_ctx, logits_out); });
}
static int bark_b200_gpt_step_batch_impl(struct bark_context * ctx, int which, int B, const int32_t * slots, const int32_t * tokens, int * n_past, float * logits_out) {
    if (!ctx || which < 0 || which > 1 || B < 1 || B > kMaxBatch || !slots || !tokens || !n_past || !logits_out) return 0;
    int top = 0;
    for (int r = 0; r < B; r++) {
        if (slots[r] < 0 || slots[r] >= kMaxBatch) return 0;
        for (int q = 0; q < r; q++) if (slots[q] == slots[r]) { fprintf(stderr, "%s: slot %d appears twice\n", __func__, slots[r]); return 0; }
        top = std::max(top, slots[r] + 1);
    }
    BARK_CUDA_CHECK(cudaSetDevice(ctx->device));
    if (!ensure_batch_slots(ctx, top)) return 0;
    GPTModel & m = *pick(ctx, which);
    float * sk[kMaxBatch], * sv[kMaxBatch];
    for (int r = 0; r < B; r++) { sk[r] = ctx->batch.k[which][slots[r]]; sv[r] = ctx->batch.v[which][slots[r]]; }
    if (!gpt_step_batch(ctx, m, B, sk, sv, tokens, n_past, 0, 0, ctx->batch.d_logits)) return 0;
    const size_t nb = (size_t) B * m.n_out_vocab * 4;
    BARK_CUDA_CHECK(cudaMemcpyAsync(logits_out, ctx->batch.d_logits, nb, cudaMemcpyDeviceToHost, ctx->stream)); g_d2h_bytes += nb;
    BARK_CUDA_CHECK(cudaStreamSynchronize(ctx->stream));
    for (int r = 0; r < B; r++) n_past[r]++;
    return 1;
}
extern "C" int bark_b200_gpt_step_batch(struct bark_context * ctx, int which, int B, const int32_t * slots, const int32_t * tokens, int * n_past, float * logits_out) {
    return guarded((int) 0, [&] { return bark_b200_gpt_step_batch_impl(ctx, which, B, slots, tokens, n_past, logits_out); });
}

extern "C" const char * bark_b200_version(void) { return "bark_b200 r3 (sm_90a; parity path + opt-in wgmma fast mode)"; }
```

### bark.cpp_b200/csrc/epilogue.cuh

```cuda
#pragma once
#include "gpt_kernels.h"

namespace bark {

__device__ __forceinline__ void store_act(void * act, int wt, int gs, int m, int k, float v) {
    if (wt == W_Q4_0) { ((float *) act)[(size_t) m * gs + k] = v; return; }
    const size_t off = gm_offset(m, k, (size_t) gs);
    if (wt == W_F16) ((__half *) act)[off] = __float2half_rn(v);
    else             ((float *) act)[off] = v;
}

template <typename T> __device__ __forceinline__ void unpack16(const uint4 & u, float (&f)[16 / sizeof(T)]);
template <> __device__ __forceinline__ void unpack16<__half>(const uint4 & u, float (&f)[8]) {
    const __half2 * h = reinterpret_cast<const __half2 *>(&u);
#pragma unroll
    for (int i = 0; i < 4; i++) { const float2 t = __half22float2(h[i]); f[2 * i] = t.x; f[2 * i + 1] = t.y; }
}
template <> __device__ __forceinline__ void unpack16<float>(const uint4 & u, float (&f)[4]) {
    f[0] = __uint_as_float(u.x); f[1] = __uint_as_float(u.y); f[2] = __uint_as_float(u.z); f[3] = __uint_as_float(u.w);
}

__device__ __forceinline__ float gelu_lookup(const __half * __restrict__ tab, float x) {
    if (x <= -10.0f) return 0.0f;
    if (x >= 10.0f) return x;
    return __half2float(tab[__half_as_ushort(__float2half_rn(x))]);
}

__device__ __forceinline__ float pv_leftovers(float sum, const float * __restrict__ v, const float * __restrict__ p, int np, int n_kv, int E) {
    int i = np, r = n_kv - np;
    while (r >= 8) { for (int l = 0; l < 8; l++) sum = __fadd_rn(sum, __fmul_rn(__ldg(v + (size_t)(i + l) * E), __ldg(p + i + l))); i += 8; r -= 8; }
    if (r >= 4)    { for (int l = 0; l < 4; l++) sum = __fadd_rn(sum, __fmul_rn(__ldg(v + (size_t)(i + l) * E), __ldg(p + i + l))); i += 4; r -= 4; }
    for (; r > 0; r--, i++) sum = __fmaf_rn(__ldg(v + (size_t) i * E), __ldg(p + i), sum);
    return sum;
}

__device__ __forceinline__ void matmul_epilogue(const MatmulEpilogue & ep, int m, int o, float r) {
    switch (ep.mode) {
        case EPI_STORE: ep.out[(size_t) m * ep.ldo + o] = r; break;
        case EPI_RESID: { float * p = ep.out + (size_t) m * ep.ldo + o; *p = __fadd_rn(r, *p); } break;
        case EPI_GELU_ACT: store_act(ep.act_out, ep.act_wt, ep.act_Kp, m, o, gelu_lookup(ep.gelu_tab, r)); break;
        case EPI_QKV: {
            const int E = ep.ldo;
            if (o < E)          ep.out[(size_t) m * E + o] = r;
            else if (o < 2 * E) { ep.k_out[(size_t) m * E + (o - E)] = r;     for (int p = 0; p < ep.n_peer; p++) ep.k_peer[p][(size_t) m * E + (o - E)] = r; }
            else                { ep.v_out[(size_t) m * E + (o - 2 * E)] = r; for (int p = 0; p < ep.n_peer; p++) ep.v_peer[p][(size_t) m * E + (o - 2 * E)] = r; }
        } break;
    }
}


}
```

### bark.cpp_b200/csrc/gemm_kernels.cu

```cuda
#include "epilogue.cuh"
#include "gpt_kernels.h"

#include <string.h>

namespace bark {

namespace {

__device__ __forceinline__ uint32_t smem_u32(const void * p) { return (uint32_t) __cvta_generic_to_shared(p); }
__device__ __forceinline__ void mbar_init(uint32_t bar, uint32_t count) { asm volatile("mbarrier.init.shared::cta.b64 [%0], %1;" ::"r"(bar), "r"(count)); }
__device__ __forceinline__ void mbar_expect_tx(uint32_t bar, uint32_t bytes) { asm volatile("mbarrier.arrive.expect_tx.shared::cta.b64 _, [%0], %1;" ::"r"(bar), "r"(bytes) : "memory"); }
__device__ __forceinline__ void mbar_wait(uint32_t bar, uint32_t parity) {
    asm volatile(
        "{\n\t.reg .pred p;\n\t"
        "WAIT_%=:\n\t"
        "mbarrier.try_wait.parity.shared::cta.b64 p, [%0], %1;\n\t"
        "@p bra DONE_%=;\n\t"
        "bra WAIT_%=;\n\t"
        "DONE_%=:\n\t}" ::"r"(bar), "r"(parity) : "memory");
}
__device__ __forceinline__ void mbar_arrive(uint32_t bar) { asm volatile("mbarrier.arrive.shared::cta.b64 _, [%0];" ::"r"(bar) : "memory"); }
__device__ __forceinline__ void tma_bulk_g2s(uint32_t dst, const void * src, uint32_t bytes, uint32_t bar) {
    asm volatile("cp.async.bulk.shared::cluster.global.mbarrier::complete_tx::bytes [%0], [%1], %2, [%3];" ::"r"(dst), "l"(src), "r"(bytes), "r"(bar) : "memory");
}

template <int N, int MASK>
__device__ __forceinline__ void butterfly_stage(float (&r)[64], bool upper) {
#pragma unroll
    for (int i = 0; i < N / 2; i++) {
        const float keep = upper ? r[i + N / 2] : r[i];
        const float send = upper ? r[i] : r[i + N / 2];
        r[i] = __fadd_rn(keep, __shfl_xor_sync(0xffffffffu, send, MASK));
    }
}
__device__ __forceinline__ int butterfly_reduce64(float (&r)[64], int lane) {
    butterfly_stage<64, 16>(r, (lane & 16) != 0);
    butterfly_stage<32, 8>(r, (lane & 8) != 0);
    butterfly_stage<16, 4>(r, (lane & 4) != 0);
    butterfly_stage<8, 1>(r, (lane & 1) != 0);
    butterfly_stage<4, 2>(r, (lane & 2) != 0);
    return ((lane & 16) << 1) | ((lane & 8) << 1) | ((lane & 4) << 1) | ((lane & 1) << 2) | (lane & 2);
}

constexpr int kBM = 32, kBO = 16, kStages = 4;
constexpr int kStageBytes = (kBM + kBO) * 512;

template <typename T> struct QuadOp;
template <> struct QuadOp<__half> {
    typedef uint2 V;
    static constexpr int kGroupsPerStage = 2;
    __device__ __forceinline__ static float elem(const uint2 & u, int c) {
        const uint32_t w = c < 2 ? u.x : u.y;
        const __half2 h = *reinterpret_cast<const __half2 *>(&w);
        return (c & 1) ? __high2float(h) : __low2float(h);
    }
};
template <> struct QuadOp<float> {
    typedef uint4 V;
    static constexpr int kGroupsPerStage = 1;
    __device__ __forceinline__ static float elem(const uint4 & u, int c) { return __uint_as_float(c == 0 ? u.x : c == 1 ? u.y : c == 2 ? u.z : u.w); }
};

}

template <typename T>
__global__ void __launch_bounds__(256, 2) lane_gemm_tiled_kernel(const T * __restrict__ Wg, int K, int w_gs, int O, const T * __restrict__ act, int act_gs, int M, MatmulEpilogue ep) {
    typedef typename QuadOp<T>::V QV;
    constexpr int GPS = QuadOp<T>::kGroupsPerStage;
    constexpr int kRowB = kGmGroup * sizeof(T);
    extern __shared__ __align__(128) unsigned char smem[];
    const uint32_t full = smem_u32(smem + kStages * kStageBytes);
    int * const cnt = reinterpret_cast<int *>(smem + kStages * kStageBytes + kStages * 8);
    const int tid = threadIdx.x, lane = tid & 31, warp = tid >> 5;
    const int wm = warp >> 1, wo = warp & 1;
    const int nsteps = K >> 5;
    const int ngroups = (nsteps + 3) >> 2;
    const int nstages = (ngroups + GPS - 1) / GPS;
    const int tiles_o = (O + kBO - 1) / kBO, tiles_m = (M + kBM - 1) / kBM, n_tiles = tiles_o * tiles_m;
    const int my_tiles = ((int) blockIdx.x < n_tiles) ? (n_tiles - 1 - (int) blockIdx.x) / (int) gridDim.x + 1 : 0;
    const int total_steps = my_tiles * nstages;

    if (tid == 0) {
        for (int s = 0; s < kStages; s++) { mbar_init(full + s * 8, 1); cnt[s] = 0; }
        asm volatile("fence.mbarrier_init.release.cluster;" ::: "memory");
    }
    __syncthreads();
    auto issue = [&](int step) {
        const int ti = step / nstages, sg = step - ti * nstages;
        const int tile = blockIdx.x + ti * gridDim.x;
        const int m0 = (tile / tiles_o) * kBM, o0 = (tile % tiles_o) * kBO;
        const int slot = step % kStages;
        const uint32_t bar = full + slot * 8;
        const int g0 = sg * GPS, ng = min(GPS, ngroups - g0);
        mbar_expect_tx(bar, (uint32_t)(ng * (kBM + kBO) * kRowB));
        const uint32_t dst = smem_u32(smem + (size_t) slot * kStageBytes);
        for (int j = 0; j < ng; j++) {
            tma_bulk_g2s(dst + j * (kBM + kBO) * kRowB, act + (size_t)(g0 + j) * act_gs + (size_t) m0 * kGmGroup, kBM * kRowB, bar);
            tma_bulk_g2s(dst + j * (kBM + kBO) * kRowB + kBM * kRowB, Wg + (size_t)(g0 + j) * w_gs + (size_t) o0 * kGmGroup, kBO * kRowB, bar);
        }
    };
    if (tid == 0) for (int s0 = 0; s0 < kStages && s0 < total_steps; s0++) issue(s0);

    int step = 0;
    for (int ti = 0; ti < my_tiles; ti++) {
        const int tile = blockIdx.x + ti * gridDim.x;
        const int m0 = (tile / tiles_o) * kBM, o0 = (tile % tiles_o) * kBO;
        float acc[64];
#pragma unroll
        for (int i = 0; i < 64; i++) acc[i] = 0.0f;
        for (int sg = 0; sg < nstages; sg++, step++) {
            const int slot = step % kStages;
            mbar_wait(full + slot * 8, (uint32_t)(step / kStages) & 1);
            const unsigned char * st = smem + (size_t) slot * kStageBytes;
#pragma unroll
            for (int j = 0; j < GPS; j++) {
                const int g = sg * GPS + j;
                if (g < ngroups) {
                    const int steps = min(4, nsteps - g * 4);
                    const unsigned char * ga = st + j * (kBM + kBO) * kRowB + lane * sizeof(QV), * gw = ga + kBM * kRowB;
                    QV pa[8], pw[8];
#pragma unroll
                    for (int mi = 0; mi < 8; mi++) pa[mi] = *reinterpret_cast<const QV *>(ga + (wm * 8 + mi) * kRowB);
#pragma unroll
                    for (int oi = 0; oi < 8; oi++) pw[oi] = *reinterpret_cast<const QV *>(gw + (wo * 8 + oi) * kRowB);
#pragma unroll
                    for (int c = 0; c < 4; c++) {
                        if (c < steps) {
                            float af[8], wf[8];
#pragma unroll
                            for (int mi = 0; mi < 8; mi++) af[mi] = QuadOp<T>::elem(pa[mi], c);
#pragma unroll
                            for (int oi = 0; oi < 8; oi++) wf[oi] = QuadOp<T>::elem(pw[oi], c);
#pragma unroll
                            for (int mi = 0; mi < 8; mi++)
#pragma unroll
                                for (int oi = 0; oi < 8; oi++) acc[mi * 8 + oi] = __fmaf_rn(wf[oi], af[mi], acc[mi * 8 + oi]);
                        }
                    }
                }
            }
            __syncwarp();
            if (lane == 0) {
                __threadfence_block();
                if (atomicAdd_block(&cnt[slot], 1) == 7) {
                    cnt[slot] = 0;
                    __threadfence_block();
                    asm volatile("fence.proxy.async.shared::cta;" ::: "memory");
                    if (step + kStages < total_steps) issue(step + kStages);
                }
            }
        }
        const int base = butterfly_reduce64(acc, lane);
        const int m = m0 + wm * 8 + (base >> 3), o = o0 + wo * 8 + (base & 7);
        if (m < M) {
            if (o < O) matmul_epilogue(ep, m, o, acc[0]);
            if (o + 1 < O) matmul_epilogue(ep, m, o + 1, acc[1]);
        }
    }
}

void lane_gemm_tiled(const DMat & W, const void * act, int act_gs, int rows, const MatmulEpilogue & ep, cudaStream_t s) {
    const size_t smem = (size_t) kStages * kStageBytes + kStages * 8 + kStages * 4 + 64;
    int dev = 0, n_sm = 0;
    BARK_CUDA_CHECK(cudaGetDevice(&dev));
    BARK_CUDA_CHECK(cudaDeviceGetAttribute(&n_sm, cudaDevAttrMultiProcessorCount, dev));
    static std::atomic<unsigned long long> configured{0};
    if (first_use_on_this_device(configured)) {
        BARK_CUDA_CHECK(cudaFuncSetAttribute(lane_gemm_tiled_kernel<__half>, cudaFuncAttributeMaxDynamicSharedMemorySize, (int) smem));
        BARK_CUDA_CHECK(cudaFuncSetAttribute(lane_gemm_tiled_kernel<float>, cudaFuncAttributeMaxDynamicSharedMemorySize, (int) smem));
    }
    if (!W.p_gm) { fprintf(stderr, "bark_b200: matrix has no group-major copy for the tiled mat-mul\n"); throw std::runtime_error("unsupported configuration (see the message above)"); }
    const int n_tiles = ((W.n_out + kBO - 1) / kBO) * ((rows + kBM - 1) / kBM);
    const int grid = min(n_tiles, 2 * n_sm);
    const int w_gs = W.o_pad * kGmGroup;
    if (W.type == W_F16) BARK_LAUNCH((lane_gemm_tiled_kernel<__half>), grid, 256, smem, s, (const __half *) W.p_gm, W.K, w_gs, W.n_out, (const __half *) act, act_gs, rows, ep);
    else                 BARK_LAUNCH((lane_gemm_tiled_kernel<float>), grid, 256, smem, s, (const float *) W.p_gm, W.K, w_gs, W.n_out, (const float *) act, act_gs, rows, ep);
}

template <int DSTEPS>
__global__ void __launch_bounds__(256) attn_scores_tiled_kernel(const float * __restrict__ Q, const float * __restrict__ Kc, int N, int n_kv, int n_past, int E,
                                                                float scale, int causal, float * __restrict__ S) {
    constexpr int D = DSTEPS * 32;
    const int lane = threadIdx.x & 31, warp = threadIdx.x >> 5;
    const int h = blockIdx.z, q0 = blockIdx.y * 8, k0 = (blockIdx.x * 8 + warp) * 8;
    if (k0 >= n_kv) return;
    float qf[8][DSTEPS], kf[8][DSTEPS];
#pragma unroll
    for (int i = 0; i < 8; i++) {
        const int q = min(q0 + i, N - 1), k = min(k0 + i, n_kv - 1);
#pragma unroll
        for (int c = 0; c < DSTEPS; c++) {
            qf[i][c] = __ldg(Q + (size_t) q * E + h * D + c * 32 + lane);
            kf[i][c] = __ldg(Kc + (size_t) k * E + h * D + c * 32 + lane);
        }
    }
    float acc[64];
#pragma unroll
    for (int qi = 0; qi < 8; qi++)
#pragma unroll
        for (int ki = 0; ki < 8; ki++) {
            float a = 0.0f;
#pragma unroll
            for (int c = 0; c < DSTEPS; c++) a = __fmaf_rn(kf[ki][c], qf[qi][c], a);
            acc[qi * 8 + ki] = a;
        }
    const int base = butterfly_reduce64(acc, lane);
    const int q = q0 + (base >> 3), k = k0 + (base & 7);
    if (q < N) {
        float * row = S + ((size_t) blockIdx.z * N + q) * n_kv;
#pragma unroll
        for (int j = 0; j < 2; j++) if (k + j < n_kv) {
            float r = __fmul_rn(acc[j], scale);
            if (causal && k + j > n_past + q) r = __int_as_float(0xff800000);
            row[k + j] = r;
        }
    }
}

__global__ void __launch_bounds__(256) attn_pv_tiled_kernel(const float * __restrict__ S, const float * __restrict__ Vc, int N, int n_kv, int E, int D,
                                                            void * __restrict__ act, int wt, int Kp) {
    const int lane = threadIdx.x & 31, warp = threadIdx.x >> 5;
    const int h = blockIdx.y, q0 = blockIdx.x * 8, d0 = warp * 8;
    if (d0 >= D) return;
    const float * prow[8];
#pragma unroll
    for (int qi = 0; qi < 8; qi++) prow[qi] = S + ((size_t) h * N + min(q0 + qi, N - 1)) * n_kv;
    const float * vbase = Vc + h * D + d0;
    float acc[64];
#pragma unroll
    for (int i = 0; i < 64; i++) acc[i] = 0.0f;
    const int np = n_kv & ~31;
    for (int k = lane; k < np; k += 32) {
        const float4 v0 = __ldg(reinterpret_cast<const float4 *>(vbase + (size_t) k * E));
        const float4 v1 = __ldg(reinterpret_cast<const float4 *>(vbase + (size_t) k * E) + 1);
        const float vf[8] = {v0.x, v0.y, v0.z, v0.w, v1.x, v1.y, v1.z, v1.w};
#pragma unroll
        for (int qi = 0; qi < 8; qi++) {
            const float p = __ldg(prow[qi] + k);
#pragma unroll
            for (int di = 0; di < 8; di++) acc[qi * 8 + di] = __fmaf_rn(vf[di], p, acc[qi * 8 + di]);
        }
    }
    const int base = butterfly_reduce64(acc, lane);
    const int q = q0 + (base >> 3), d = d0 + (base & 7);
    if (q >= N) return;
    const float * p = S + ((size_t) h * N + q) * n_kv;
#pragma unroll
    for (int j = 0; j < 2; j++) {
        store_act(act, wt, Kp, q, h * D + d + j, pv_leftovers(acc[j], Vc + h * D + d + j, p, np, n_kv, E));
    }
}

void attention_tiled_scores(const float * Q, const float * Kc, int N, int n_kv, int n_past, int E, int H, float scale, bool causal, float * scores, cudaStream_t s) {
    const int D = E / H;
    const dim3 grid((n_kv + 63) / 64, (N + 7) / 8, H);
    if (D == 64)       BARK_LAUNCH(attn_scores_tiled_kernel<2>, grid, 256, 0, s, Q, Kc, N, n_kv, n_past, E, scale, causal ? 1 : 0, scores);
    else if (D == 32)  BARK_LAUNCH(attn_scores_tiled_kernel<1>, grid, 256, 0, s, Q, Kc, N, n_kv, n_past, E, scale, causal ? 1 : 0, scores);
    else if (D == 96)  BARK_LAUNCH(attn_scores_tiled_kernel<3>, grid, 256, 0, s, Q, Kc, N, n_kv, n_past, E, scale, causal ? 1 : 0, scores);
    else               BARK_LAUNCH(attn_scores_tiled_kernel<4>, grid, 256, 0, s, Q, Kc, N, n_kv, n_past, E, scale, causal ? 1 : 0, scores);
}

void attention_tiled_pv(const float * scores, const float * Vc, int N, int n_kv, int E, int H, void * act, WType wt, int Kp, cudaStream_t s) {
    const int D = E / H;
    BARK_LAUNCH(attn_pv_tiled_kernel, dim3((N + 7) / 8, H), 32 * ((D + 7) / 8), 0, s, scores, Vc, N, n_kv, E, D, act, (int) wt, Kp);
}

}
```

### bark.cpp_b200/csrc/gpt_kernels.cu

```cuda
#include "gpt_kernels.h"
#include "epilogue.cuh"

#include <cstring>

namespace bark {

std::atomic<unsigned long long> g_kernel_launches{0};

template <typename T>
__global__ void permute_to_li_kernel(const T * __restrict__ src, T * __restrict__ dst, int n_out, int K, int Kp) {
    constexpr int G = 16 / sizeof(T);
    const size_t total = (size_t) n_out * Kp;
    for (size_t i = (size_t) blockIdx.x * blockDim.x + threadIdx.x; i < total; i += (size_t) gridDim.x * blockDim.x) {
        const int o = (int)(i / Kp), j = (int)(i % Kp);
        const int e = j % G, gv = j / G, v = gv % 32, g = gv / 32;
        const int k = (g * G + e) * 32 + v;
        dst[i] = (k < K) ? src[(size_t) o * K + k] : T(0);
    }
}

void permute_to_li(const void * src, void * dst, int n_out, int K, WType t, cudaStream_t s) {
    if (t == W_F16) { const int Kp = li_padded_k(K, 2); BARK_LAUNCH(permute_to_li_kernel<__half>, 1184, 256, 0, s, (const __half *) src, (__half *) dst, n_out, K, Kp); }
    else            { const int Kp = li_padded_k(K, 4); BARK_LAUNCH(permute_to_li_kernel<float>, 1184, 256, 0, s, (const float *) src, (float *) dst, n_out, K, Kp); }
}

template <typename T>
__global__ void permute_to_gm_kernel(const T * __restrict__ src, T * __restrict__ dst, int n_out, int o_pad, int K) {
    const size_t gs = (size_t) o_pad * kGmGroup, total = (size_t) gm_groups(K) * gs;
    for (size_t i = (size_t) blockIdx.x * blockDim.x + threadIdx.x; i < total; i += (size_t) gridDim.x * blockDim.x) {
        const int g = (int)(i / gs), r = (int)(i % gs), o = r / kGmGroup, w = r % kGmGroup, v = w >> 2, c = w & 3;
        const int k = g * kGmGroup + c * 32 + v;
        dst[i] = (o < n_out && k < K) ? src[(size_t) o * K + k] : T(0);
    }
}

void permute_to_gm(const void * src, void * dst, int n_out, int o_pad, int K, WType t, cudaStream_t s) {
    if (t == W_F16) BARK_LAUNCH(permute_to_gm_kernel<__half>, 1184, 256, 0, s, (const __half *) src, (__half *) dst, n_out, o_pad, K);
    else            BARK_LAUNCH(permute_to_gm_kernel<float>, 1184, 256, 0, s, (const float *) src, (float *) dst, n_out, o_pad, K);
}

__device__ __forceinline__ float wte_value(const void * wte, int wt, int E, int row, int i) {
    if (wt == W_F16) return __half2float(((const __half *) wte)[(size_t) row * E + i]);
    if (wt == W_Q4_0) {
        const unsigned char * blk = (const unsigned char *) wte + ((size_t) row * (E >> 5) + (i >> 5)) * 18;
        const float d = __half2float(__ushort_as_half((unsigned short)(blk[0] | (blk[1] << 8))));
        const int j = i & 31, q = j < 16 ? (blk[2 + j] & 0x0f) : (blk[2 + j - 16] >> 4);
        return __fmul_rn((float)(q - 8), d);
    }
    return ((const float *) wte)[(size_t) row * E + i];
}

__global__ void embed_causal_kernel(const void * __restrict__ wte, int wt, const float * __restrict__ wpe, const int32_t * __restrict__ tok,
                                    int N, int n_past, int merge, int E, float * __restrict__ x, const int32_t * __restrict__ pos) {
    const int r = blockIdx.x;
    for (int i = threadIdx.x; i < E; i += blockDim.x) {
        float v;
        if (merge) {
            if (r < 256) v = __fadd_rn(wte_value(wte, wt, E, tok[r], i), wte_value(wte, wt, E, tok[256 + r], i));
            else         v = wte_value(wte, wt, E, tok[512], i);
        } else {
            v = wte_value(wte, wt, E, tok[r], i);
        }
        x[(size_t) r * E + i] = __fadd_rn(v, wpe[(size_t)(pos ? pos[r] : r + n_past) * E + i]);
    }
}

struct FineTables { const void * wte[8]; };
__global__ void embed_fine_kernel(FineTables tabs, int wt, const float * __restrict__ wpe, const int32_t * __restrict__ ids ,
                                  int nn, int E, float * __restrict__ x, int row0) {
    const int r = row0 + blockIdx.x;
    for (int i = threadIdx.x; i < E; i += blockDim.x) {
        float v = 0.0f;
        for (int c = 0; c <= nn; c++) v = __fadd_rn(v, wte_value(tabs.wte[c], wt, E, ids[c * 1024 + r], i));
        x[(size_t) blockIdx.x * E + i] = __fadd_rn(v, wpe[(size_t) r * E + i]);
    }
}

void gpt_embed_causal(const GPTModel & m, const int32_t * d_tok, int N, int n_past, bool merge, float * x, cudaStream_t s, const int32_t * d_pos) {
    if (qx_supported(m.wtype)) { qx_embed_causal(m, d_tok, N, n_past, merge, x, s, d_pos); return; }
    BARK_LAUNCH(embed_causal_kernel, N, 256, 0, s, m.wte[0], (int) m.wtype, m.wpe, d_tok, N, n_past, merge ? 1 : 0, m.n_embd, x, d_pos);
}
void gpt_embed_fine(const GPTModel & m, const int32_t * d_ids, int nn, float * x, cudaStream_t s, int row0, int rows) {
    if (qx_supported(m.wtype)) { qx_embed_fine(m, d_ids, nn, x, s); return; }
    FineTables t; for (int i = 0; i < 8; i++) t.wte[i] = m.wte[i];
    BARK_LAUNCH(embed_fine_kernel, rows, 256, 0, s, t, (int) m.wtype, m.wpe, d_ids, nn, m.n_embd, x, row0);
}

__device__ __forceinline__ double warp_sum_d(double v) {
#pragma unroll
    for (int o = 16; o > 0; o >>= 1) v += __shfl_xor_sync(0xffffffffu, v, o);
    return v;
}

__global__ void layernorm_act_kernel(const float * __restrict__ x, int rows, int E, const float * __restrict__ g, const float * __restrict__ b,
                                     void * __restrict__ act, int wt, int Kp, float eps, unsigned * __restrict__ fallback_counter) {
    const int warp = (blockIdx.x * blockDim.x + threadIdx.x) >> 5, lane = threadIdx.x & 31;
    if (warp >= rows) return;
    const float * xr = x + (size_t) warp * E;
    const double slack = 2.0 * (double) E * 0x1p-53 * (1.0 + 1e-6);

    double s = 0.0, a = 0.0;
    for (int i = lane; i < E; i += 32) { const double v = (double) xr[i]; s += v; a += fabs(v); }
    s = warp_sum_d(s); a = warp_sum_d(a);
    double d = slack * a;
    float mean = __double2float_rn(__ddiv_rn(s, (double) E));
    if (__double2float_rn(__ddiv_rn(s - d, (double) E)) != __double2float_rn(__ddiv_rn(s + d, (double) E))) {
        double ss = 0.0;
        if (lane == 0) { for (int i = 0; i < E; i++) ss = __dadd_rn(ss, (double) xr[i]); if (fallback_counter) atomicAdd(fallback_counter, 1u); }
        ss = __shfl_sync(0xffffffffu, ss, 0);
        mean = __double2float_rn(__ddiv_rn(ss, (double) E));
    }

    double s2 = 0.0;
    for (int i = lane; i < E; i += 32) { const float v = __fsub_rn(xr[i], mean); s2 += (double) __fmul_rn(v, v); }
    s2 = warp_sum_d(s2);
    d = slack * s2;
    float variance = __double2float_rn(__ddiv_rn(s2, (double) E));
    if (__double2float_rn(__ddiv_rn(s2 - d, (double) E)) != __double2float_rn(__ddiv_rn(s2 + d, (double) E))) {
        double ss = 0.0;
        if (lane == 0) { for (int i = 0; i < E; i++) { const float v = __fsub_rn(xr[i], mean); ss = __dadd_rn(ss, (double) __fmul_rn(v, v)); } if (fallback_counter) atomicAdd(fallback_counter, 1u); }
        ss = __shfl_sync(0xffffffffu, ss, 0);
        variance = __double2float_rn(__ddiv_rn(ss, (double) E));
    }
    const float scale = __fdiv_rn(1.0f, __fsqrt_rn(__fadd_rn(variance, eps)));
    for (int i = lane; i < E; i += 32) {
        float y = __fmul_rn(__fsub_rn(xr[i], mean), scale);
        y = __fmul_rn(y, g[i]);
        if (b) y = __fadd_rn(y, b[i]);
        store_act(act, wt, Kp, warp, i, y);
    }
}

void layernorm_act(const float * x, int rows, int E, const float * g, const float * b, void * act, WType wt, int Kp, unsigned * fallback_counter, cudaStream_t s) {
    const int warps_per_block = 8;
    BARK_LAUNCH(layernorm_act_kernel, (rows + warps_per_block - 1) / warps_per_block, warps_per_block * 32, 0, s, x, rows, E, g, b, act, (int) wt, Kp, 1e-5f, fallback_counter);
}

template <typename T> struct Quad;
template <> struct Quad<__half> {
    typedef uint2 V;
    __device__ static void unpack(const uint2 & u, float (&f)[4]) {
        const float2 a = __half22float2(*reinterpret_cast<const __half2 *>(&u.x)), b = __half22float2(*reinterpret_cast<const __half2 *>(&u.y));
        f[0] = a.x; f[1] = a.y; f[2] = b.x; f[3] = b.y;
    }
};
template <> struct Quad<float> {
    typedef uint4 V;
    __device__ static void unpack(const uint4 & u, float (&f)[4]) { f[0] = __uint_as_float(u.x); f[1] = __uint_as_float(u.y); f[2] = __uint_as_float(u.z); f[3] = __uint_as_float(u.w); }
};

template <typename T, int MT>
__global__ void __launch_bounds__(256) lane_matmul_kernel(const T * __restrict__ W, int K, int Kp, int O, const T * __restrict__ act, int act_gs, int M, MatmulEpilogue ep) {
    constexpr int G = 16 / sizeof(T), QPG = G / 4;
    typedef typename Quad<T>::V QV;
    const int lane = threadIdx.x & 31, warp = threadIdx.x >> 5;
    const int o = blockIdx.x * 8 + warp;
    const int m0 = blockIdx.y * MT;
    if (o >= O) return;
    const int nsteps = K >> 5;
    const int ngroups = (nsteps + G - 1) / G;
    const uint4 * wrow = reinterpret_cast<const uint4 *>(W + (size_t) o * Kp) + lane;
    const QV * arow[MT];
    int mvalid = 0;
#pragma unroll
    for (int mi = 0; mi < MT; mi++) { const int m = min(m0 + mi, M - 1); arow[mi] = reinterpret_cast<const QV *>(act + (size_t) m * kGmGroup) + lane; if (m0 + mi < M) mvalid = mi + 1; }
    const size_t qstride = (size_t) act_gs * sizeof(T) / sizeof(QV);
    float acc[MT];
#pragma unroll
    for (int mi = 0; mi < MT; mi++) acc[mi] = 0.0f;
    for (int g = 0; g < ngroups; g++) {
        const int steps = min(G, nsteps - g * G);
        float w[G]; unpack16<T>(__ldg(wrow + g * 32), w);
#pragma unroll
        for (int mi = 0; mi < MT; mi++) {
#pragma unroll
            for (int qd = 0; qd < QPG; qd++) {
                if (qd * 4 < steps) {
                    float a[4]; Quad<T>::unpack(__ldg(arow[mi] + (size_t)(g * QPG + qd) * qstride), a);
#pragma unroll
                    for (int e = 0; e < 4; e++) if (qd * 4 + e < steps) acc[mi] = __fmaf_rn(w[qd * 4 + e], a[e], acc[mi]);
                }
            }
        }
    }
#pragma unroll
    for (int mi = 0; mi < MT; mi++) {
        const float r = lane_tree_reduce(acc[mi]);
        if (lane == 0 && mi < mvalid) matmul_epilogue(ep, m0 + mi, o, r);
    }
}

static bool use_tiled() { static const bool t = [] { const char * e = getenv("BARK_B200_GEMM"); return !(e && !strcmp(e, "simple")); }(); return t; }

void lane_matmul(const DMat & W, const void * act, int act_gs, int rows, const MatmulEpilogue & ep, cudaStream_t s) {
    if (W.type == W_Q4_0) { q4_matmul(W, act, act_gs, rows, ep, s); return; }
    if (qx_supported(W.type)) { qx_matmul(W, act, act_gs, rows, ep, s); return; }
    const int gx = (W.n_out + 7) / 8;
    {
        const double es = W.type == W_F16 ? 2.0 : 4.0;
        g_next_bytes = (double) W.n_out * W.K * es + (double) rows * (W.K * es + W.n_out * 4.0);
        g_next_flops = 2.0 * rows * (double) W.n_out * W.K;
    }
    if (rows >= 16 && use_tiled() && (W.type == W_F16 || W.type == W_F32)) { lane_gemm_tiled(W, act, act_gs, rows, ep, s); return; }
    if (W.type == W_F16) {
        if (rows == 1) BARK_LAUNCH((lane_matmul_kernel<__half, 1>), dim3(gx, 1), 256, 0, s, (const __half *) W.p, W.K, W.Kp, W.n_out, (const __half *) act, act_gs, rows, ep);
        else           BARK_LAUNCH((lane_matmul_kernel<__half, 8>), dim3(gx, (rows + 7) / 8), 256, 0, s, (const __half *) W.p, W.K, W.Kp, W.n_out, (const __half *) act, act_gs, rows, ep);
    } else if (W.type == W_F32) {
        if (rows == 1) BARK_LAUNCH((lane_matmul_kernel<float, 1>), dim3(gx, 1), 256, 0, s, (const float *) W.p, W.K, W.Kp, W.n_out, (const float *) act, act_gs, rows, ep);
        else           BARK_LAUNCH((lane_matmul_kernel<float, 8>), dim3(gx, (rows + 7) / 8), 256, 0, s, (const float *) W.p, W.K, W.Kp, W.n_out, (const float *) act, act_gs, rows, ep);
    } else {
        fprintf(stderr, "bark_b200: q4_0 mul_mat is not built in this revision\n"); throw std::runtime_error("unsupported configuration (see the message above)");
    }
}

template <int DSTEPS>
__global__ void attn_scores_kernel(const float * __restrict__ Q, const float * __restrict__ Kc, int N, int n_kv, int n_past, int E, int H,
                                   float scale, int causal, float * __restrict__ S) {
    const int D = DSTEPS * 32;
    const int lane = threadIdx.x & 31;
    const int wq = blockIdx.x * (blockDim.x >> 5) + (threadIdx.x >> 5);
    if (wq >= H * N) return;
    const int h = wq / N, q = wq % N;
    float qv[DSTEPS];
#pragma unroll
    for (int c = 0; c < DSTEPS; c++) qv[c] = Q[(size_t) q * E + h * D + c * 32 + lane];
    float * srow = S + ((size_t) h * N + q) * n_kv;
    for (int k = 0; k < n_kv; k++) {
        const float * kr = Kc + (size_t) k * E + h * D;
        float acc = 0.0f;
#pragma unroll
        for (int c = 0; c < DSTEPS; c++) acc = __fmaf_rn(kr[c * 32 + lane], qv[c], acc);
        float r = lane_tree_reduce(acc);
        r = __fmul_rn(r, scale);
        if (causal && k > n_past + q) r = __int_as_float(0xff800000);
        if (lane == (k & 31)) srow[k] = r;
    }
}

__device__ __forceinline__ void softmax_row(float * __restrict__ p, int n_kv) {
    const int lane = threadIdx.x & 31;
    float mx = __int_as_float(0xff800000);
    for (int i = lane; i < n_kv; i += 32) mx = fmaxf(mx, p[i]);
#pragma unroll
    for (int o = 16; o > 0; o >>= 1) mx = fmaxf(mx, __shfl_xor_sync(0xffffffffu, mx, o));
    const int nchunks = n_kv >> 3;
    float csum[4] = {0.f, 0.f, 0.f, 0.f};
#pragma unroll
    for (int slot = 0; slot < 4; slot++) {
        const int c = slot * 32 + lane;
        if (c < nchunks) {
            float v[8];
#pragma unroll
            for (int l = 0; l < 8; l++) { v[l] = ggml_v_expf_dev(__fsub_rn(p[c * 8 + l], mx)); }
#pragma unroll
            for (int l = 0; l < 8; l++) p[c * 8 + l] = v[l];
            const float t0 = __fadd_rn(v[4], v[0]), t1 = __fadd_rn(v[5], v[1]), t2 = __fadd_rn(v[6], v[2]), t3 = __fadd_rn(v[7], v[3]);
            csum[slot] = __fadd_rn(__fadd_rn(t0, t2), __fadd_rn(t1, t3));
        }
    }
    for (int i = nchunks * 8; i < n_kv; i++) {
        const float val = glibc_expf_dev(__fsub_rn(p[i], mx));
        if (lane == 0) p[i] = val;
    }
    __syncwarp();
    double tsum = 0.0;
#pragma unroll
    for (int slot = 0; slot < 4; slot++) tsum += (double) csum[slot];
#pragma unroll
    for (int o = 16; o > 0; o >>= 1) tsum += __shfl_xor_sync(0xffffffffu, tsum, o);
    float sc;
    {
        const double dl = 2.0 * (double)(nchunks + 8) * 0x1p-53 * tsum * (1.0 + 1e-6);
        double lo = tsum - dl, hi = tsum + dl;
        for (int i = nchunks * 8; i < n_kv; i++) { const double tl = (double) p[i]; lo = __dadd_rn(lo, tl); hi = __dadd_rn(hi, tl); }
        const double mid = 0.5 * (lo + hi);
        double y = (double) __frcp_rn((float) mid);
        double e = __fma_rn(-mid, y, 1.0); y = __fma_rn(y, e, y);
        e = __fma_rn(-mid, y, 1.0);        y = __fma_rn(y, e, y);
        const double rw = (hi - lo) * y * 0.5 + 0x1p-48;
        sc = __double2float_rn(y * (1.0 - rw));
        if (sc != __double2float_rn(y * (1.0 + rw))) {
            double sum = 0.0;
#pragma unroll
            for (int slot = 0; slot < 4; slot++) {
                const int base = slot * 32;
                if (base < nchunks) {
                    const int cnt = min(32, nchunks - base);
                    for (int l = 0; l < cnt; l++) sum = __dadd_rn(sum, (double) __shfl_sync(0xffffffffu, csum[slot], l));
                }
            }
            for (int i = nchunks * 8; i < n_kv; i++) sum = __dadd_rn(sum, (double) p[i]);
            sc = __double2float_rn(__ddiv_rn(1.0, sum));
        }
    }
    __syncwarp();
    for (int i = lane; i < n_kv; i += 32) p[i] = __fmul_rn(p[i], sc);
}

__global__ void attn_softmax_kernel(float * __restrict__ S, int rows, int n_kv) {
    const int row = blockIdx.x * (blockDim.x >> 5) + (threadIdx.x >> 5);
    if (row >= rows) return;
    softmax_row(S + (size_t) row * n_kv, n_kv);
}

__global__ void attn_pv_kernel(const float * __restrict__ S, const float * __restrict__ Vc, int N, int n_kv, int E, int H, int D,
                               void * __restrict__ act, int wt, int Kp) {
    const int d = threadIdx.x, q = blockIdx.x * blockDim.y + threadIdx.y, h = blockIdx.y;
    if (q >= N || d >= D) return;
    const float * p = S + ((size_t) h * N + q) * n_kv;
    const float * v = Vc + h * D + d;
    float acc[32];
#pragma unroll
    for (int l = 0; l < 32; l++) acc[l] = 0.0f;
    const int np = n_kv & ~31;
    for (int k0 = 0; k0 < np; k0 += 32) {
#pragma unroll
        for (int l = 0; l < 32; l++) acc[l] = __fmaf_rn(v[(size_t)(k0 + l) * E], p[k0 + l], acc[l]);
    }
    store_act(act, wt, Kp, q, h * D + d, pv_leftovers(lane_tree_reduce_local(acc), v, p, np, n_kv, E));
}

__device__ __forceinline__ float * row_cache(float * const (&p)[8], int b) {
    float * r = p[0];
#pragma unroll
    for (int i = 1; i < 8; i++) if (b == i) r = p[i];
    return r;
}

template <int DSTEPS>
__global__ void __launch_bounds__(256) attn_scores_batch_kernel(const float * __restrict__ Q, const float * __restrict__ Kst, const float * __restrict__ Vst,
                                                                BatchKV kv, const int32_t * __restrict__ pos, int E, int ld_s, float scale, float * __restrict__ S) {
    constexpr int D = DSTEPS * 32;
    const int lane = threadIdx.x & 31, warp = threadIdx.x >> 5;
    const int h = blockIdx.y, b = blockIdx.z, last = pos[b];
    float * const Kc = row_cache(kv.k, b);
    if (blockIdx.x == 0) {
        float * const Vc = row_cache(kv.v, b);
        for (int i = threadIdx.x; i < D; i += blockDim.x) {
            Kc[(size_t) last * E + h * D + i] = Kst[(size_t) b * E + h * D + i];
            Vc[(size_t) last * E + h * D + i] = Vst[(size_t) b * E + h * D + i];
        }
    }
    const int k0 = (blockIdx.x * 8 + warp) * 8;
    if (k0 > last) return;
    float qv[DSTEPS], kf[8][DSTEPS];
#pragma unroll
    for (int c = 0; c < DSTEPS; c++) qv[c] = __ldg(Q + (size_t) b * E + h * D + c * 32 + lane);
#pragma unroll
    for (int i = 0; i < 8; i++) {
        const int k = min(k0 + i, last);
        const float * kr = (k == last ? Kst + (size_t) b * E : Kc + (size_t) k * E) + h * D;
#pragma unroll
        for (int c = 0; c < DSTEPS; c++) kf[i][c] = kr[c * 32 + lane];
    }
    float * srow = S + ((size_t) b * gridDim.y + h) * ld_s;
#pragma unroll
    for (int i = 0; i < 8; i++) {
        float acc = 0.0f;
#pragma unroll
        for (int c = 0; c < DSTEPS; c++) acc = __fmaf_rn(kf[i][c], qv[c], acc);
        const float r = lane_tree_reduce(acc);
        if (lane == 0 && k0 + i <= last) srow[k0 + i] = __fmul_rn(r, scale);
    }
}

__global__ void attn_softmax_batch_kernel(float * __restrict__ S, int rows, int H, int ld_s, const int32_t * __restrict__ pos) {
    const int row = blockIdx.x * (blockDim.x >> 5) + (threadIdx.x >> 5);
    if (row >= rows) return;
    softmax_row(S + (size_t) row * ld_s, pos[row / H] + 1);
}

__global__ void __launch_bounds__(32) attn_pv_batch_kernel(const float * __restrict__ S, BatchKV kv, const int32_t * __restrict__ pos, int E, int D, int ld_s,
                                                           void * __restrict__ act, int wt, int Kp) {
    const int lane = threadIdx.x & 31;
    const int h = blockIdx.y, b = blockIdx.z, d0 = blockIdx.x * 8;
    const int n_kv = pos[b] + 1, np = n_kv & ~31;
    const float * p = S + ((size_t) b * gridDim.y + h) * ld_s;
    const float * vbase = row_cache(kv.v, b) + h * D + d0;
    float acc[8];
#pragma unroll
    for (int j = 0; j < 8; j++) acc[j] = 0.0f;
#pragma unroll 4
    for (int k = lane; k < np; k += 32) {
        const float4 v0 = __ldg(reinterpret_cast<const float4 *>(vbase + (size_t) k * E));
        const float4 v1 = __ldg(reinterpret_cast<const float4 *>(vbase + (size_t) k * E) + 1);
        const float pk = __ldg(p + k);
        acc[0] = __fmaf_rn(v0.x, pk, acc[0]); acc[1] = __fmaf_rn(v0.y, pk, acc[1]); acc[2] = __fmaf_rn(v0.z, pk, acc[2]); acc[3] = __fmaf_rn(v0.w, pk, acc[3]);
        acc[4] = __fmaf_rn(v1.x, pk, acc[4]); acc[5] = __fmaf_rn(v1.y, pk, acc[5]); acc[6] = __fmaf_rn(v1.z, pk, acc[6]); acc[7] = __fmaf_rn(v1.w, pk, acc[7]);
    }
    float mine = 0.0f;
#pragma unroll
    for (int j = 0; j < 8; j++) { const float r = lane_tree_reduce(acc[j]); if (lane == j) mine = r; }
    if (lane < 8) store_act(act, wt, Kp, b, h * D + d0 + lane, pv_leftovers(mine, vbase + lane, p, np, n_kv, E));
}

void attention_batch(const float * Q, const float * Kst, const float * Vst, const BatchKV & kv, const int32_t * d_pos, int B, int max_kv, int E, int H,
                     float * scores, void * act, WType wt, int Kp, cudaStream_t s) {
    const int D = E / H;
    const float scale = 1.0f / sqrtf((float) E / (float) H);
    const dim3 grid((max_kv + 63) / 64, H, B);
    g_next_bytes = 4.0 * B * ((double) max_kv * E + 3.0 * E + (double) H * max_kv); g_next_flops = 2.0 * B * (double) max_kv * E;
    if (D == 64)       BARK_LAUNCH(attn_scores_batch_kernel<2>, grid, 256, 0, s, Q, Kst, Vst, kv, d_pos, E, max_kv, scale, scores);
    else if (D == 32)  BARK_LAUNCH(attn_scores_batch_kernel<1>, grid, 256, 0, s, Q, Kst, Vst, kv, d_pos, E, max_kv, scale, scores);
    else if (D == 96)  BARK_LAUNCH(attn_scores_batch_kernel<3>, grid, 256, 0, s, Q, Kst, Vst, kv, d_pos, E, max_kv, scale, scores);
    else if (D == 128) BARK_LAUNCH(attn_scores_batch_kernel<4>, grid, 256, 0, s, Q, Kst, Vst, kv, d_pos, E, max_kv, scale, scores);
    else { fprintf(stderr, "bark_b200: unsupported head size %d (need a multiple of 32, <= 128)\n", D); throw std::runtime_error("unsupported configuration (see the message above)"); }
    g_next_bytes = 8.0 * B * H * (double) max_kv;
    BARK_LAUNCH(attn_softmax_batch_kernel, (B * H + 7) / 8, 256, 0, s, scores, B * H, H, max_kv, d_pos);
    g_next_bytes = 4.0 * B * ((double) max_kv * E + (double) H * max_kv + E); g_next_flops = 2.0 * B * (double) max_kv * E;
    BARK_LAUNCH(attn_pv_batch_kernel, dim3(D / 8, H, B), 32, 0, s, scores, kv, d_pos, E, D, max_kv, act, (int) wt, Kp);
}

void attention(const float * Q, const float * Kc, const float * Vc, int N, int n_kv, int n_past, int E, int H, bool causal,
               float * scores, void * act, WType wt, int Kp, cudaStream_t s) {
    const int D = E / H;
    const float scale = 1.0f / sqrtf((float) E / (float) H);
    const int rows = H * N;
    if (use_tiled() && D % 32 == 0 && D <= 128) {
        g_next_bytes = 4.0 * ((double) n_kv * E + (double) N * E + (double) H * N * n_kv); g_next_flops = 2.0 * (double) N * n_kv * E;
        attention_tiled_scores(Q, Kc, N, n_kv, n_past, E, H, scale, causal, scores, s);
        g_next_bytes = 8.0 * (double) rows * n_kv;
        BARK_LAUNCH(attn_softmax_kernel, (rows + 7) / 8, 256, 0, s, scores, rows, n_kv);
        g_next_bytes = 4.0 * ((double) n_kv * E + (double) H * N * n_kv + (double) N * E); g_next_flops = 2.0 * (double) N * n_kv * E;
        attention_tiled_pv(scores, Vc, N, n_kv, E, H, act, wt, Kp, s);
        return;
    }
    g_next_bytes = 4.0 * ((double) n_kv * E + (double) N * E + (double) H * N * n_kv); g_next_flops = 2.0 * (double) N * n_kv * E;
    if (D == 64)       BARK_LAUNCH(attn_scores_kernel<2>, (rows + 7) / 8, 256, 0, s, Q, Kc, N, n_kv, n_past, E, H, scale, causal ? 1 : 0, scores);
    else if (D == 32)  BARK_LAUNCH(attn_scores_kernel<1>, (rows + 7) / 8, 256, 0, s, Q, Kc, N, n_kv, n_past, E, H, scale, causal ? 1 : 0, scores);
    else if (D == 96)  BARK_LAUNCH(attn_scores_kernel<3>, (rows + 7) / 8, 256, 0, s, Q, Kc, N, n_kv, n_past, E, H, scale, causal ? 1 : 0, scores);
    else if (D == 128) BARK_LAUNCH(attn_scores_kernel<4>, (rows + 7) / 8, 256, 0, s, Q, Kc, N, n_kv, n_past, E, H, scale, causal ? 1 : 0, scores);
    else { fprintf(stderr, "bark_b200: unsupported head size %d (need a multiple of 32, <= 128)\n", D); throw std::runtime_error("unsupported configuration (see the message above)"); }
    g_next_bytes = 8.0 * (double) rows * n_kv;
    BARK_LAUNCH(attn_softmax_kernel, (rows + 7) / 8, 256, 0, s, scores, rows, n_kv);
    const int qy = max(1, 256 / D);
    g_next_bytes = 4.0 * ((double) n_kv * E + (double) H * N * n_kv + (double) N * E); g_next_flops = 2.0 * (double) N * n_kv * E;
    BARK_LAUNCH(attn_pv_kernel, dim3((N + qy - 1) / qy, H), dim3(D, qy), 0, s, scores, Vc, N, n_kv, E, H, D, act, (int) wt, Kp);
}

}
```

### bark.cpp_b200/csrc/gpt_kernels.h

```cpp
#pragma once
#include "model.h"

namespace bark {

enum EpiMode : int { EPI_STORE = 0, EPI_RESID = 1, EPI_GELU_ACT = 2, EPI_QKV = 3 };

struct MatmulEpilogue {
    int mode = EPI_STORE;
    float * out = nullptr; int ldo = 0;
    float * k_out = nullptr, * v_out = nullptr;
    int n_peer = 0; float * k_peer[7] = {nullptr}, * v_peer[7] = {nullptr};
    void * act_out = nullptr; int act_wt = 0, act_Kp = 0;
    const __half * gelu_tab = nullptr;
};

void permute_to_li(const void * src_rowmajor, void * dst_li, int n_out, int K, WType t, cudaStream_t s);
void permute_to_gm(const void * src_rowmajor, void * dst_gm, int n_out, int o_pad, int K, WType t, cudaStream_t s);

void gpt_embed_causal(const GPTModel & m, const int32_t * d_tok, int N, int n_past, bool merge, float * x, cudaStream_t s, const int32_t * d_pos = nullptr);
void gpt_embed_fine(const GPTModel & m, const int32_t * d_ids, int nn, float * x, cudaStream_t s, int row0 = 0, int rows = 1024);

void layernorm_act(const float * x, int rows, int E, const float * g, const float * b, void * act, WType wt, int Kp,
                   unsigned * fallback_counter, cudaStream_t s);

void lane_matmul(const DMat & W, const void * act, int act_gs, int rows, const MatmulEpilogue & ep, cudaStream_t s);

void attention(const float * Q, const float * Kc, const float * Vc, int N, int n_kv, int n_past, int E, int H, bool causal,
               float * scores, void * act, WType wt, int Kp, cudaStream_t s);

struct BatchKV { float * k[8], * v[8]; };
void attention_batch(const float * Q, const float * Kst, const float * Vst, const BatchKV & kv, const int32_t * d_pos, int B, int max_kv, int E, int H,
                     float * scores, void * act, WType wt, int Kp, cudaStream_t s);

void q4_split(const void * raw_blocks, size_t n_blocks, void * qs, void * scales, cudaStream_t s);
void q4_set_scratch(void * q8, void * q8_scales);
void q4_matmul(const DMat & W, const void * act_f32, int ld_act, int rows, const MatmulEpilogue & ep, cudaStream_t s);

bool   qx_supported(WType t);
size_t qx_block_bytes(WType t);
void   qx_split(const void * raw_blocks, size_t n_blocks, WType t, void * qs, void * qh, void * d, void * m, cudaStream_t s);
void   qx_set_scratch(void * q8, void * q8_scales, void * q8_sums);
void   qx_embed_causal(const GPTModel & m, const int32_t * d_tok, int N, int n_past, bool merge, float * x, cudaStream_t s, const int32_t * d_pos);
void   qx_embed_fine(const GPTModel & m, const int32_t * d_ids, int nn, float * x, cudaStream_t s);
void   qx_matmul(const DMat & W, const void * act_f32, int ld_act, int rows, const MatmulEpilogue & ep, cudaStream_t s);

void lane_gemm_tiled(const DMat & W, const void * act, int act_gs, int rows, const MatmulEpilogue & ep, cudaStream_t s);
void attention_tiled_scores(const float * Q, const float * Kc, int N, int n_kv, int n_past, int E, int H, float scale, bool causal, float * scores, cudaStream_t s);
void attention_tiled_pv(const float * scores, const float * Vc, int N, int n_kv, int E, int H, void * act, WType wt, int Kp, cudaStream_t s);

enum { FEPI_F32 = 0, FEPI_RESID = 1, FEPI_GELU16 = 2, FEPI_QKV16 = 4 };
struct FastEpi {
    int mode = FEPI_F32;
    float * out32 = nullptr; __half * out16 = nullptr; int ldo = 0;
    __half * vt = nullptr; int vt_ld = 0, v_col0 = 0;
};
int  fast_gemm(const __half * A, int lda, const __half * W, int ldw, int M, int N, int K, const FastEpi & ep, int n_sm, int bn, cudaStream_t s);
bool fast_attention(const __half * qk, int ldq, int k_col0, const __half * vt, int n, int E, int H, __half * out, cudaStream_t s);
void fast_layernorm(const float * x, int rows, int E, const float * g, const float * b, __half * out, cudaStream_t s);

constexpr int kDecodeReplicas = 8;
struct DecodePhase { const void * w; int n_out, row_bytes, K, pad; const void * ws; };
struct DecodeLayerVec { const float * ln_1_g, * ln_1_b, * ln_2_g, * ln_2_b; };
struct DecodeArgs {
    const DecodePhase * phases;
    const DecodeLayerVec * layer_vecs;
    const void * wte; const float * wpe; const float * ln_f_g, * ln_f_b; const __half * gelu_tab;
    float * mem_k, * mem_v;
    unsigned long long * gx, * gq, * gk, * gv, * gatt, * gff, * gscores;
    float * logits;
    unsigned tag_base; unsigned * ln_fallbacks;
    unsigned long long * timing;
    int E, H, L, block_size, n_past, token, lm_lo, lm_hi;
    const int32_t * token_ptr; int n_vocab_in;
    double inv_E;
    unsigned headstart[6];
    int timing_tid; unsigned poll_ns;
};
int  decode_tags_per_step(int n_layer);
void launch_decode_step(const DecodeArgs & args, WType wt, int n_sm, cudaStream_t s);
bool decode_cluster_supported(const DecodeArgs & args, WType wt, int max_row_bytes);
void launch_decode_cluster(const DecodeArgs & args, WType wt, cudaStream_t s);

}
```

### include/bark_b200.h

```cpp
#pragma once
#include "bark.h"

#ifdef __cplusplus
extern "C" {
#endif

BARK_API void bark_b200_set_device(int cuda_device);
BARK_API const char * bark_b200_version(void);

BARK_API int  bark_b200_gpt_eval(struct bark_context * ctx, int which, const int32_t * tokens, int n, int * n_past, int merge_ctx, float * logits_out);
BARK_API int  bark_b200_fine_eval(struct bark_context * ctx, const int32_t * in_buffer, int nn, float * logits_out);
BARK_API int  bark_b200_encodec_decode(struct bark_context * ctx, const int32_t * codes, int n_frames, float * out, int out_cap);
BARK_API int  bark_b200_sample(struct bark_context * ctx, int which, const float * logits, int n, float temp, float * eos_p);
BARK_API int  bark_b200_sample_rows(struct bark_context * ctx, const float * logits , int n, int rows, float temp, int32_t * tokens_out,
                                     float * eos_p_out );
BARK_API void bark_b200_reseed(struct bark_context * ctx, uint32_t seed);
BARK_API void bark_b200_tokenize(struct bark_context * ctx, const char * text, int32_t * out513);

BARK_API bool bark_b200_forward_text_encoder(struct bark_context * ctx, int n_threads);
BARK_API bool bark_b200_forward_coarse_encoder(struct bark_context * ctx, int n_threads);
BARK_API bool bark_b200_forward_fine_encoder(struct bark_context * ctx, int n_threads);

BARK_API int  bark_b200_get_tokens(struct bark_context * ctx, int stage, int32_t * out, int cap);
BARK_API void bark_b200_set_tokens(struct bark_context * ctx, int stage, const int32_t * in, int n);
BARK_API void bark_b200_get_stats(struct bark_context * ctx, struct bark_statistics * out, int64_t * per_model9);
BARK_API void bark_b200_get_hparams(struct bark_context * ctx, int which, int32_t * out10);
BARK_API unsigned long long bark_b200_kernel_launches(void);
BARK_API unsigned bark_b200_layernorm_fallbacks(struct bark_context * ctx);

BARK_API void bark_b200_profile_enable(int on);
BARK_API int  bark_b200_profile_report(char * buf, int cap);
BARK_API void bark_b200_io_counters(unsigned long long * h2d_bytes, unsigned long long * d2h_bytes, int reset);
BARK_API int  bark_b200_decode_timing(struct bark_context * ctx, unsigned long long * out, int n);


BARK_API int  bark_b200_shard_init(struct bark_context * ctx, int rank, int world, void * handle_out);
BARK_API int  bark_b200_shard_connect(struct bark_context * ctx, const void * all_handles);
BARK_API unsigned long long bark_b200_shard_nvlink_bytes(struct bark_context * ctx, int reset);

BARK_API bool bark_b200_generate_batch(struct bark_context * ctx, const char * const * texts, const uint32_t * seeds, int n, int n_threads);
BARK_API int  bark_b200_batch_audio(struct bark_context * ctx, int i, float * out, int cap);
BARK_API int  bark_b200_batch_tokens(struct bark_context * ctx, int i, int stage, int32_t * out, int cap);
BARK_API int  bark_b200_gpt_eval_slot(struct bark_context * ctx, int which, int slot, const int32_t * tokens, int n, int * n_past, int merge_ctx, float * logits_out);
BARK_API int  bark_b200_gpt_step_batch(struct bark_context * ctx, int which, int B, const int32_t * slots, const int32_t * tokens, int * n_past, float * logits_out);

BARK_API int  bark_b200_fast_mode(struct bark_context * ctx);
BARK_API int  bark_b200_fast_gemm(const uint16_t * A, const uint16_t * W, void * C, int M, int N, int K, int epilogue, int bn);
BARK_API int  bark_b200_fast_attention(const uint16_t * q, const uint16_t * k, const uint16_t * v, uint16_t * out, int n, int E, int H);

#ifdef __cplusplus
}
#endif
```

Measured before the change: 11.47.

## Fuse attention scores, softmax and PV into one tiled kernel

```diff
diff --git a/bark.cpp_b200/__init__.py b/bark.cpp_b200/__init__.py
--- a/bark.cpp_b200/__init__.py
+++ b/bark.cpp_b200/__init__.py
@@ -38,7 +38,7 @@
     "bark_b200_get_stats", "bark_b200_get_hparams", "bark_b200_kernel_launches", "bark_b200_layernorm_fallbacks",
     "bark_b200_profile_enable", "bark_b200_profile_report", "bark_b200_io_counters", "bark_b200_decode_timing",
     "bark_b200_shard_init", "bark_b200_shard_connect", "bark_b200_shard_nvlink_bytes",
-    "bark_b200_fast_mode", "bark_b200_fast_gemm", "bark_b200_fast_attention",
+    "bark_b200_fast_mode", "bark_b200_fast_gemm", "bark_b200_fast_attention", "bark_b200_parity_attention",
     "bark_b200_generate_batch", "bark_b200_batch_audio", "bark_b200_batch_tokens", "bark_b200_gpt_eval_slot", "bark_b200_gpt_step_batch",
     "ggml_time_init", "ggml_time_us", "ggml_time_ms", "ggml_init", "ggml_free",
 ]
@@ -114,6 +114,8 @@
     L.bark_b200_fast_gemm.argtypes = [vp, vp, vp, C.c_int, C.c_int, C.c_int, C.c_int, C.c_int]
     L.bark_b200_fast_attention.restype = C.c_int
     L.bark_b200_fast_attention.argtypes = [vp, vp, vp, vp, C.c_int, C.c_int, C.c_int]
+    L.bark_b200_parity_attention.restype = C.c_int
+    L.bark_b200_parity_attention.argtypes = [vp, vp, vp, vp] + [C.c_int] * 7
     L.bark_b200_generate_batch.restype = C.c_bool
     L.bark_b200_generate_batch.argtypes = [vp, C.POINTER(C.c_char_p), C.POINTER(C.c_uint32), C.c_int, C.c_int]
     L.bark_b200_batch_audio.restype = C.c_int
@@ -358,6 +360,20 @@
     return out
 
 
+ATTN_PATHS = {"auto": 0, "fused": 1, "tiled": 2}
+
+
+def parity_attention(q: np.ndarray, k: np.ndarray, v: np.ndarray, n_head: int, n_past: int = 0, causal: bool = False, path: str = "auto") -> np.ndarray:
+    q, k, v = (np.ascontiguousarray(a, np.float32) for a in (q, k, v))
+    N, E = q.shape
+    n_kv = k.shape[0]
+    assert k.shape == v.shape == (n_kv, E), (q.shape, k.shape, v.shape)
+    out = np.zeros((N, E), np.float32)
+    if not lib().bark_b200_parity_attention(_p(q), _p(k), _p(v), _p(out), N, n_kv, n_past, E, n_head, int(causal), ATTN_PATHS[path]):
+        raise RuntimeError("bark_b200_parity_attention failed")
+    return out
+
+
 def kernel_launches() -> int:
     return int(lib().bark_b200_kernel_launches())
 
diff --git a/bark.cpp_b200/csrc/bark_api.cu b/bark.cpp_b200/csrc/bark_api.cu
--- a/bark.cpp_b200/csrc/bark_api.cu
+++ b/bark.cpp_b200/csrc/bark_api.cu
@@ -591,9 +591,9 @@
 }
 
 void alloc_workspace(bark_context * ctx) {
-    int E = 0, H = 0; size_t kp_bytes = 0, n_logits = 0;
+    int E = 0, H = 0, max_block = 0; size_t kp_bytes = 0, n_logits = 0;
     for (GPTModel * m : {&ctx->semantic, &ctx->coarse, &ctx->fine}) {
-        E = std::max(E, (int) m->n_embd); H = std::max(H, (int) m->n_head);
+        E = std::max(E, (int) m->n_embd); H = std::max(H, (int) m->n_head); max_block = std::max(max_block, (int) m->block_size);
         const size_t es = m->wtype == W_F16 ? 2 : 4;
         kp_bytes = std::max(kp_bytes, (size_t) li_padded_k(4 * m->n_embd, (int) es) * es);
     }
@@ -607,7 +607,7 @@
     ws.q    = (float *) ctx_alloc(ctx, R * E * 4);
     ws.kbuf = (float *) ctx_alloc(ctx, R * E * 4);
     ws.vbuf = (float *) ctx_alloc(ctx, R * E * 4);
-    ws.scores = (float *) ctx_alloc(ctx, (size_t) H * R * R * 4);
+    ws.scores = (float *) ctx_alloc(ctx, std::max((size_t) 8 * max_block, (size_t) attn_tiled_max_rows(H, ctx->n_sm_total) * 1024) * H * 4);
     ws.logits = (float *) ctx_alloc(ctx, n_logits * 4);
     ws.tok  = (int32_t *) ctx_alloc(ctx, 8 * 1024 * 4);
     if (is_quant(ctx->semantic.wtype) || is_quant(ctx->coarse.wtype) || is_quant(ctx->fine.wtype)) {
@@ -929,6 +929,38 @@
 }
 extern "C" int bark_b200_fast_attention(const uint16_t * q, const uint16_t * k, const uint16_t * v, uint16_t * out, int n, int E, int H) { return guarded((int) 0, [&] { return bark_b200_fast_attention_impl(q, k, v, out, n, E, H); }); }
 extern "C" int bark_b200_fast_mode(struct bark_context * ctx) { return ctx && ctx->fast_mode ? 1 : 0; }
+static int bark_b200_parity_attention_impl(const float * q, const float * k, const float * v, float * out, int N, int n_kv, int n_past, int E, int H,
+                                           int causal, int path) {
+    if (!q || !k || !v || !out || N < 1 || n_kv < 1 || n_kv > 1024 || n_past < 0 || H < 1 || E % H || path < 0 || path > 2) return 0;
+    const int D = E / H;
+    if (D % 32 || D > 128) return 0;
+    struct Buffers {
+        float * p[5] = {nullptr, nullptr, nullptr, nullptr, nullptr};
+        ~Buffers() { for (float * b : p) cudaFree(b); }
+    } d;
+    float *& dq = d.p[0], *& dk = d.p[1], *& dv = d.p[2], *& dout = d.p[3], *& dsc = d.p[4];
+    BARK_CUDA_CHECK(cudaMalloc(&dq, (size_t) N * E * 4)); BARK_CUDA_CHECK(cudaMalloc(&dk, (size_t) n_kv * E * 4));
+    BARK_CUDA_CHECK(cudaMalloc(&dv, (size_t) n_kv * E * 4)); BARK_CUDA_CHECK(cudaMalloc(&dout, (size_t) N * E * 4));
+    BARK_CUDA_CHECK(cudaMalloc(&dsc, (size_t) H * N * n_kv * 4));
+    BARK_CUDA_CHECK(cudaMemcpy(dq, q, (size_t) N * E * 4, cudaMemcpyHostToDevice)); BARK_CUDA_CHECK(cudaMemcpy(dk, k, (size_t) n_kv * E * 4, cudaMemcpyHostToDevice));
+    BARK_CUDA_CHECK(cudaMemcpy(dv, v, (size_t) n_kv * E * 4, cudaMemcpyHostToDevice));
+    BARK_CUDA_CHECK(cudaMemset(dout, 0xff, (size_t) N * E * 4));
+    if (path == ATTN_TILED) {
+        int dev = 0, n_sm = 0;
+        BARK_CUDA_CHECK(cudaGetDevice(&dev)); BARK_CUDA_CHECK(cudaDeviceGetAttribute(&n_sm, cudaDevAttrMultiProcessorCount, dev));
+        if (N > attn_tiled_max_rows(H, n_sm)) return 0;
+    }
+    attention(dq, dk, dv, N, n_kv, n_past, E, H, causal != 0, dsc, dout, W_Q4_0, E, 0, (AttnPath) path);
+    BARK_CUDA_CHECK(cudaGetLastError());
+    const cudaError_t e = cudaDeviceSynchronize();
+    if (e != cudaSuccess) { fprintf(stderr, "bark_b200_parity_attention: %s\n", cudaGetErrorString(e)); return 0; }
+    BARK_CUDA_CHECK(cudaMemcpy(out, dout, (size_t) N * E * 4, cudaMemcpyDeviceToHost));
+    return 1;
+}
+extern "C" int bark_b200_parity_attention(const float * q, const float * k, const float * v, float * out, int N, int n_kv, int n_past, int E, int H, int causal,
+                                          int path) {
+    return guarded((int) 0, [&] { return bark_b200_parity_attention_impl(q, k, v, out, N, n_kv, n_past, E, H, causal, path); });
+}
 
 extern "C" bool bark_b200_generate_batch(struct bark_context * ctx, const char * const * texts, const uint32_t * seeds, int n, int n_threads) {
     (void) n_threads;
diff --git a/bark.cpp_b200/csrc/epilogue.cuh b/bark.cpp_b200/csrc/epilogue.cuh
--- a/bark.cpp_b200/csrc/epilogue.cuh
+++ b/bark.cpp_b200/csrc/epilogue.cuh
@@ -26,11 +26,71 @@
     return __half2float(tab[__half_as_ushort(__float2half_rn(x))]);
 }
 
+__device__ __forceinline__ void softmax_row(float * __restrict__ p, int n_kv) {
+    const int lane = threadIdx.x & 31;
+    float mx = __int_as_float(0xff800000);
+    for (int i = lane; i < n_kv; i += 32) mx = fmaxf(mx, p[i]);
+#pragma unroll
+    for (int o = 16; o > 0; o >>= 1) mx = fmaxf(mx, __shfl_xor_sync(0xffffffffu, mx, o));
+    const int nchunks = n_kv >> 3;
+    float csum[4] = {0.f, 0.f, 0.f, 0.f};
+#pragma unroll
+    for (int slot = 0; slot < 4; slot++) {
+        const int c = slot * 32 + lane;
+        if (c < nchunks) {
+            float v[8];
+#pragma unroll
+            for (int l = 0; l < 8; l++) { v[l] = ggml_v_expf_dev(__fsub_rn(p[c * 8 + l], mx)); }
+#pragma unroll
+            for (int l = 0; l < 8; l++) p[c * 8 + l] = v[l];
+            const float t0 = __fadd_rn(v[4], v[0]), t1 = __fadd_rn(v[5], v[1]), t2 = __fadd_rn(v[6], v[2]), t3 = __fadd_rn(v[7], v[3]);
+            csum[slot] = __fadd_rn(__fadd_rn(t0, t2), __fadd_rn(t1, t3));
+        }
+    }
+    for (int i = nchunks * 8; i < n_kv; i++) {
+        const float val = glibc_expf_dev(__fsub_rn(p[i], mx));
+        if (lane == 0) p[i] = val;
+    }
+    __syncwarp();
+    double tsum = 0.0;
+#pragma unroll
+    for (int slot = 0; slot < 4; slot++) tsum += (double) csum[slot];
+#pragma unroll
+    for (int o = 16; o > 0; o >>= 1) tsum += __shfl_xor_sync(0xffffffffu, tsum, o);
+    float sc;
+    {
+        const double dl = 2.0 * (double)(nchunks + 8) * 0x1p-53 * tsum * (1.0 + 1e-6);
+        double lo = tsum - dl, hi = tsum + dl;
+        for (int i = nchunks * 8; i < n_kv; i++) { const double tl = (double) p[i]; lo = __dadd_rn(lo, tl); hi = __dadd_rn(hi, tl); }
+        const double mid = 0.5 * (lo + hi);
+        double y = (double) __frcp_rn((float) mid);
+        double e = __fma_rn(-mid, y, 1.0); y = __fma_rn(y, e, y);
+        e = __fma_rn(-mid, y, 1.0);        y = __fma_rn(y, e, y);
+        const double rw = (hi - lo) * y * 0.5 + 0x1p-48;
+        sc = __double2float_rn(y * (1.0 - rw));
+        if (sc != __double2float_rn(y * (1.0 + rw))) {
+            double sum = 0.0;
+#pragma unroll
+            for (int slot = 0; slot < 4; slot++) {
+                const int base = slot * 32;
+                if (base < nchunks) {
+                    const int cnt = min(32, nchunks - base);
+                    for (int l = 0; l < cnt; l++) sum = __dadd_rn(sum, (double) __shfl_sync(0xffffffffu, csum[slot], l));
+                }
+            }
+            for (int i = nchunks * 8; i < n_kv; i++) sum = __dadd_rn(sum, (double) p[i]);
+            sc = __double2float_rn(__ddiv_rn(1.0, sum));
+        }
+    }
+    __syncwarp();
+    for (int i = lane; i < n_kv; i += 32) p[i] = __fmul_rn(p[i], sc);
+}
+
 __device__ __forceinline__ float pv_leftovers(float sum, const float * __restrict__ v, const float * __restrict__ p, int np, int n_kv, int E) {
     int i = np, r = n_kv - np;
-    while (r >= 8) { for (int l = 0; l < 8; l++) sum = __fadd_rn(sum, __fmul_rn(__ldg(v + (size_t)(i + l) * E), __ldg(p + i + l))); i += 8; r -= 8; }
-    if (r >= 4)    { for (int l = 0; l < 4; l++) sum = __fadd_rn(sum, __fmul_rn(__ldg(v + (size_t)(i + l) * E), __ldg(p + i + l))); i += 4; r -= 4; }
-    for (; r > 0; r--, i++) sum = __fmaf_rn(__ldg(v + (size_t) i * E), __ldg(p + i), sum);
+    while (r >= 8) { for (int l = 0; l < 8; l++) sum = __fadd_rn(sum, __fmul_rn(v[(size_t)(i + l) * E], p[i + l])); i += 8; r -= 8; }
+    if (r >= 4)    { for (int l = 0; l < 4; l++) sum = __fadd_rn(sum, __fmul_rn(v[(size_t)(i + l) * E], p[i + l])); i += 4; r -= 4; }
+    for (; r > 0; r--, i++) sum = __fmaf_rn(v[(size_t) i * E], p[i], sum);
     return sum;
 }
 
diff --git a/bark.cpp_b200/csrc/gemm_kernels.cu b/bark.cpp_b200/csrc/gemm_kernels.cu
--- a/bark.cpp_b200/csrc/gemm_kernels.cu
+++ b/bark.cpp_b200/csrc/gemm_kernels.cu
@@ -1,6 +1,7 @@
 #include "epilogue.cuh"
 #include "gpt_kernels.h"
 
+#include <algorithm>
 #include <string.h>
 
 namespace bark {
@@ -177,6 +178,134 @@
     else                 BARK_LAUNCH((lane_gemm_tiled_kernel<float>), grid, 256, smem, s, (const float *) W.p_gm, W.K, w_gs, W.n_out, (const float *) act, act_gs, rows, ep);
 }
 
+constexpr int kAttnQ = 32, kAttnKT = 64, kAttnVK = 512, kAttnVW = 16;
+constexpr int kAttnVLd = kAttnVW + 4;
+
+__host__ __device__ inline int attn_ld(int n_kv) { return ((n_kv + 31) & ~31) + 1; }
+__host__ __device__ inline int attn_ring_off(int n_kv) { return (kAttnQ * attn_ld(n_kv) + 3) & ~3; }
+
+namespace {
+__device__ __forceinline__ void cp_async_16(void * dst, const float * src) { asm volatile("cp.async.cg.shared.global [%0], [%1], 16;" ::"r"(smem_u32(dst)), "l"(src) : "memory"); }
+__device__ __forceinline__ void cp_async_commit() { asm volatile("cp.async.commit_group;" ::: "memory"); }
+__device__ __forceinline__ void cp_async_wait_prev() { asm volatile("cp.async.wait_group 1;" ::: "memory"); }
+}
+
+template <int DSTEPS>
+__global__ void __launch_bounds__(256, 1) attn_fused_kernel(const float * __restrict__ Q, const float * __restrict__ Kc, const float * __restrict__ Vc,
+                                                            int N, int n_kv, int n_past, int E, float scale, int causal,
+                                                            void * __restrict__ act, int wt, int Kp) {
+    constexpr int D = DSTEPS * 32;
+    extern __shared__ __align__(16) float sm[];
+    const int tid = threadIdx.x, lane = tid & 31, warp = tid >> 5;
+    const int h = blockIdx.y, q0 = blockIdx.x * kAttnQ;
+    const int ld = attn_ld(n_kv);
+    float * const P = sm;
+    float * const ring = sm + attn_ring_off(n_kv);
+    const float * const kh = Kc + h * D, * const vh = Vc + h * D;
+    const float ninf = __int_as_float(0xff800000);
+
+    float qr[D];
+    {
+        const float4 * qrow = reinterpret_cast<const float4 *>(Q + (size_t) min(q0 + lane, N - 1) * E + h * D);
+#pragma unroll
+        for (int i = 0; i < D / 4; i++) { const float4 t = __ldg(qrow + i); qr[4 * i] = t.x; qr[4 * i + 1] = t.y; qr[4 * i + 2] = t.z; qr[4 * i + 3] = t.w; }
+    }
+    const int n_kt = (n_kv + kAttnKT - 1) / kAttnKT;
+    auto issue_k = [&](int t) {
+        if (t < n_kt) {
+            float * const dst = ring + (t & 1) * kAttnKT * D;
+            for (int i = tid; i < kAttnKT * D / 4; i += 256) {
+                const int r = i / (D / 4), c = i % (D / 4), k = t * kAttnKT + r;
+                if (k < n_kv) cp_async_16(dst + r * D + c * 4, kh + (size_t) k * E + c * 4);
+            }
+        }
+        cp_async_commit();
+    };
+    issue_k(0); issue_k(1);
+    const int k_vis = n_past + min(q0 + kAttnQ, N) - 1;
+    for (int t = 0; t < n_kt; t++) {
+        cp_async_wait_prev();
+        __syncthreads();
+        const float * const kt = ring + (t & 1) * kAttnKT * D;
+        for (int j = 0; j < 8; j++) {
+            const int kl = warp * 8 + j, k = t * kAttnKT + kl;
+            if (k >= n_kv) break;
+            float r = ninf;
+            if (!causal || k <= k_vis) {
+                float a[32];
+#pragma unroll
+                for (int v = 0; v < 32; v++) a[v] = 0.0f;
+#pragma unroll
+                for (int c = 0; c < DSTEPS; c++)
+#pragma unroll
+                    for (int v4 = 0; v4 < 8; v4++) {
+                        const float4 kk = *reinterpret_cast<const float4 *>(kt + kl * D + c * 32 + v4 * 4);
+                        a[v4 * 4]     = __fmaf_rn(kk.x, qr[c * 32 + v4 * 4],     a[v4 * 4]);
+                        a[v4 * 4 + 1] = __fmaf_rn(kk.y, qr[c * 32 + v4 * 4 + 1], a[v4 * 4 + 1]);
+                        a[v4 * 4 + 2] = __fmaf_rn(kk.z, qr[c * 32 + v4 * 4 + 2], a[v4 * 4 + 2]);
+                        a[v4 * 4 + 3] = __fmaf_rn(kk.w, qr[c * 32 + v4 * 4 + 3], a[v4 * 4 + 3]);
+                    }
+                r = __fmul_rn(lane_tree_reduce_local(a), scale);
+                if (causal && k > n_past + q0 + lane) r = ninf;
+            }
+            P[lane * ld + k] = r;
+        }
+        __syncthreads();
+        issue_k(t + 2);
+    }
+
+    const int np = n_kv & ~31;
+    const int vk = min(kAttnVK, np), n_ch = vk ? (np + vk - 1) / vk : 0;
+    auto issue_v = [&](int i) {
+        if (i < n_ch * (D / kAttnVW)) {
+            const int rd = i / n_ch, k0 = (i % n_ch) * vk, rows = min(vk, np - k0);
+            float * const dst = ring + (i & 1) * vk * kAttnVLd;
+            for (int e = tid; e < rows * 4; e += 256)
+                cp_async_16(dst + (e >> 2) * kAttnVLd + (e & 3) * 4, vh + (size_t)(k0 + (e >> 2)) * E + rd * kAttnVW + (e & 3) * 4);
+        }
+        cp_async_commit();
+    };
+    issue_v(0); issue_v(1);
+
+    for (int r = warp; r < min(kAttnQ, N - q0); r += 8) softmax_row(P + r * ld, n_kv);
+    __syncthreads();
+
+    const int qs = warp & 3, cs = warp >> 2;
+    const float * const pw = P + qs * 8 * ld;
+    int i = 0;
+    for (int rd = 0; rd < D / kAttnVW; rd++) {
+        float acc[64];
+#pragma unroll
+        for (int a = 0; a < 64; a++) acc[a] = 0.0f;
+        for (int c = 0; c < n_ch; c++, i++) {
+            const int k0 = c * vk, rows = min(vk, np - k0);
+            cp_async_wait_prev();
+            __syncthreads();
+            const float * const vt = ring + (i & 1) * vk * kAttnVLd + cs * 8;
+            for (int kl = lane; kl < rows; kl += 32) {
+                const float4 v0 = *reinterpret_cast<const float4 *>(vt + kl * kAttnVLd);
+                const float4 v1 = *reinterpret_cast<const float4 *>(vt + kl * kAttnVLd + 4);
+                const float vf[8] = {v0.x, v0.y, v0.z, v0.w, v1.x, v1.y, v1.z, v1.w};
+#pragma unroll
+                for (int qi = 0; qi < 8; qi++) {
+                    const float p = pw[qi * ld + k0 + kl];
+#pragma unroll
+                    for (int di = 0; di < 8; di++) acc[qi * 8 + di] = __fmaf_rn(vf[di], p, acc[qi * 8 + di]);
+                }
+            }
+            __syncthreads();
+            issue_v(i + 2);
+        }
+        const int base = butterfly_reduce64(acc, lane);
+        const int q = q0 + qs * 8 + (base >> 3), d = rd * kAttnVW + cs * 8 + (base & 7);
+        if (q < N) {
+            const float * const p = P + (q - q0) * ld;
+#pragma unroll
+            for (int j = 0; j < 2; j++) store_act(act, wt, Kp, q, h * D + d + j, pv_leftovers(acc[j], vh + d + j, p, np, n_kv, E));
+        }
+    }
+}
+
 template <int DSTEPS>
 __global__ void __launch_bounds__(256) attn_scores_tiled_kernel(const float * __restrict__ Q, const float * __restrict__ Kc, int N, int n_kv, int n_past, int E,
                                                                 float scale, int causal, float * __restrict__ S) {
@@ -217,7 +346,7 @@
     }
 }
 
-__global__ void __launch_bounds__(256) attn_pv_tiled_kernel(const float * __restrict__ S, const float * __restrict__ Vc, int N, int n_kv, int E, int D,
+__global__ void __launch_bounds__(512) attn_pv_tiled_kernel(const float * __restrict__ S, const float * __restrict__ Vc, int N, int n_kv, int E, int D,
                                                             void * __restrict__ act, int wt, int Kp) {
     const int lane = threadIdx.x & 31, warp = threadIdx.x >> 5;
     const int h = blockIdx.y, q0 = blockIdx.x * 8, d0 = warp * 8;
@@ -251,18 +380,60 @@
     }
 }
 
-void attention_tiled_scores(const float * Q, const float * Kc, int N, int n_kv, int n_past, int E, int H, float scale, bool causal, float * scores, cudaStream_t s) {
+__global__ void attn_softmax_kernel(float * __restrict__ S, int rows, int n_kv) {
+    const int row = blockIdx.x * (blockDim.x >> 5) + (threadIdx.x >> 5);
+    if (row >= rows) return;
+    softmax_row(S + (size_t) row * n_kv, n_kv);
+}
+
+int attn_tiled_max_rows(int H, int n_sm) { return kAttnQ * ((n_sm + H - 1) / H - 1); }
+
+void attention(const float * Q, const float * Kc, const float * Vc, int N, int n_kv, int n_past, int E, int H, bool causal,
+               float * scores, void * act, WType wt, int Kp, cudaStream_t s, AttnPath path) {
     const int D = E / H;
-    const dim3 grid((n_kv + 63) / 64, (N + 7) / 8, H);
-    if (D == 64)       BARK_LAUNCH(attn_scores_tiled_kernel<2>, grid, 256, 0, s, Q, Kc, N, n_kv, n_past, E, scale, causal ? 1 : 0, scores);
-    else if (D == 32)  BARK_LAUNCH(attn_scores_tiled_kernel<1>, grid, 256, 0, s, Q, Kc, N, n_kv, n_past, E, scale, causal ? 1 : 0, scores);
-    else if (D == 96)  BARK_LAUNCH(attn_scores_tiled_kernel<3>, grid, 256, 0, s, Q, Kc, N, n_kv, n_past, E, scale, causal ? 1 : 0, scores);
-    else               BARK_LAUNCH(attn_scores_tiled_kernel<4>, grid, 256, 0, s, Q, Kc, N, n_kv, n_past, E, scale, causal ? 1 : 0, scores);
-}
-
-void attention_tiled_pv(const float * scores, const float * Vc, int N, int n_kv, int E, int H, void * act, WType wt, int Kp, cudaStream_t s) {
-    const int D = E / H;
-    BARK_LAUNCH(attn_pv_tiled_kernel, dim3((N + 7) / 8, H), 32 * ((D + 7) / 8), 0, s, scores, Vc, N, n_kv, E, D, act, (int) wt, Kp);
-}
-
-}
+    if (E % H || D < 32 || D % 32 || D > 128 || N < 1 || n_kv < 1 || n_kv > 1024) {
+        fprintf(stderr, "bark_b200: attention needs a head size of 32, 64, 96 or 128 and 1..1024 keys (got %d heads of %d, %d keys)\n", H, D, n_kv);
+        throw std::runtime_error("unsupported configuration (see the message above)");
+    }
+    const float scale = 1.0f / sqrtf((float) E / (float) H);
+    int dev = 0, n_sm = 0;
+    BARK_CUDA_CHECK(cudaGetDevice(&dev));
+    BARK_CUDA_CHECK(cudaDeviceGetAttribute(&n_sm, cudaDevAttrMultiProcessorCount, dev));
+    if (path == ATTN_TILED || (path == ATTN_AUTO && N <= attn_tiled_max_rows(H, n_sm))) {
+        if (N > attn_tiled_max_rows(H, n_sm)) {
+            fprintf(stderr, "bark_b200: %d rows exceed the score buffer of the three-kernel attention (%d)\n", N, attn_tiled_max_rows(H, n_sm));
+            throw std::runtime_error("unsupported configuration (see the message above)");
+        }
+        const int rows = H * N, c = causal ? 1 : 0;
+        const dim3 grid((n_kv + 63) / 64, (N + 7) / 8, H);
+        g_next_bytes = 4.0 * ((double) n_kv * E + (double) N * E + (double) H * N * n_kv); g_next_flops = 2.0 * (double) N * n_kv * E;
+        if (D == 64)      BARK_LAUNCH(attn_scores_tiled_kernel<2>, grid, 256, 0, s, Q, Kc, N, n_kv, n_past, E, scale, c, scores);
+        else if (D == 32) BARK_LAUNCH(attn_scores_tiled_kernel<1>, grid, 256, 0, s, Q, Kc, N, n_kv, n_past, E, scale, c, scores);
+        else if (D == 96) BARK_LAUNCH(attn_scores_tiled_kernel<3>, grid, 256, 0, s, Q, Kc, N, n_kv, n_past, E, scale, c, scores);
+        else              BARK_LAUNCH(attn_scores_tiled_kernel<4>, grid, 256, 0, s, Q, Kc, N, n_kv, n_past, E, scale, c, scores);
+        g_next_bytes = 8.0 * (double) rows * n_kv;
+        BARK_LAUNCH(attn_softmax_kernel, (rows + 7) / 8, 256, 0, s, scores, rows, n_kv);
+        g_next_bytes = 4.0 * ((double) n_kv * E + (double) H * N * n_kv + (double) N * E); g_next_flops = 2.0 * (double) N * n_kv * E;
+        BARK_LAUNCH(attn_pv_tiled_kernel, dim3((N + 7) / 8, H), 32 * ((D + 7) / 8), 0, s, scores, Vc, N, n_kv, E, D, act, (int) wt, Kp);
+        return;
+    }
+    const int np = n_kv & ~31;
+    const size_t ring = std::max((size_t) 2 * kAttnKT * D, (size_t) 2 * std::min(kAttnVK, np) * kAttnVLd);
+    const size_t smem = ((size_t) attn_ring_off(n_kv) + ring) * 4;
+    static std::atomic<unsigned long long> configured{0};
+    if (first_use_on_this_device(configured)) {
+        const size_t most = ((size_t) attn_ring_off(1024) + std::max(2 * kAttnKT * 128, 2 * kAttnVK * kAttnVLd)) * 4;
+        BARK_CUDA_CHECK(cudaFuncSetAttribute(attn_fused_kernel<1>, cudaFuncAttributeMaxDynamicSharedMemorySize, (int) most));
+        BARK_CUDA_CHECK(cudaFuncSetAttribute(attn_fused_kernel<2>, cudaFuncAttributeMaxDynamicSharedMemorySize, (int) most));
+        BARK_CUDA_CHECK(cudaFuncSetAttribute(attn_fused_kernel<3>, cudaFuncAttributeMaxDynamicSharedMemorySize, (int) most));
+        BARK_CUDA_CHECK(cudaFuncSetAttribute(attn_fused_kernel<4>, cudaFuncAttributeMaxDynamicSharedMemorySize, (int) most));
+    }
+    const dim3 grid((N + kAttnQ - 1) / kAttnQ, H);
+    g_next_bytes = 4.0 * (2.0 * N * E + 2.0 * n_kv * E); g_next_flops = 4.0 * N * (double) n_kv * E;
+    const int c = causal ? 1 : 0;
+    if (D == 64)      BARK_LAUNCH(attn_fused_kernel<2>, grid, 256, smem, s, Q, Kc, Vc, N, n_kv, n_past, E, scale, c, act, (int) wt, Kp);
+    else if (D == 32) BARK_LAUNCH(attn_fused_kernel<1>, grid, 256, smem, s, Q, Kc, Vc, N, n_kv, n_past, E, scale, c, act, (int) wt, Kp);
+    else if (D == 96) BARK_LAUNCH(attn_fused_kernel<3>, grid, 256, smem, s, Q, Kc, Vc, N, n_kv, n_past, E, scale, c, act, (int) wt, Kp);
+    else              BARK_LAUNCH(attn_fused_kernel<4>, grid, 256, smem, s, Q, Kc, Vc, N, n_kv, n_past, E, scale, c, act, (int) wt, Kp);
+}
+}
diff --git a/bark.cpp_b200/csrc/gpt_kernels.cu b/bark.cpp_b200/csrc/gpt_kernels.cu
--- a/bark.cpp_b200/csrc/gpt_kernels.cu
+++ b/bark.cpp_b200/csrc/gpt_kernels.cu
@@ -211,113 +211,6 @@
     } else {
         fprintf(stderr, "bark_b200: q4_0 mul_mat is not built in this revision\n"); throw std::runtime_error("unsupported configuration (see the message above)");
     }
-}
-
-template <int DSTEPS>
-__global__ void attn_scores_kernel(const float * __restrict__ Q, const float * __restrict__ Kc, int N, int n_kv, int n_past, int E, int H,
-                                   float scale, int causal, float * __restrict__ S) {
-    const int D = DSTEPS * 32;
-    const int lane = threadIdx.x & 31;
-    const int wq = blockIdx.x * (blockDim.x >> 5) + (threadIdx.x >> 5);
-    if (wq >= H * N) return;
-    const int h = wq / N, q = wq % N;
-    float qv[DSTEPS];
-#pragma unroll
-    for (int c = 0; c < DSTEPS; c++) qv[c] = Q[(size_t) q * E + h * D + c * 32 + lane];
-    float * srow = S + ((size_t) h * N + q) * n_kv;
-    for (int k = 0; k < n_kv; k++) {
-        const float * kr = Kc + (size_t) k * E + h * D;
-        float acc = 0.0f;
-#pragma unroll
-        for (int c = 0; c < DSTEPS; c++) acc = __fmaf_rn(kr[c * 32 + lane], qv[c], acc);
-        float r = lane_tree_reduce(acc);
-        r = __fmul_rn(r, scale);
-        if (causal && k > n_past + q) r = __int_as_float(0xff800000);
-        if (lane == (k & 31)) srow[k] = r;
-    }
-}
-
-__device__ __forceinline__ void softmax_row(float * __restrict__ p, int n_kv) {
-    const int lane = threadIdx.x & 31;
-    float mx = __int_as_float(0xff800000);
-    for (int i = lane; i < n_kv; i += 32) mx = fmaxf(mx, p[i]);
-#pragma unroll
-    for (int o = 16; o > 0; o >>= 1) mx = fmaxf(mx, __shfl_xor_sync(0xffffffffu, mx, o));
-    const int nchunks = n_kv >> 3;
-    float csum[4] = {0.f, 0.f, 0.f, 0.f};
-#pragma unroll
-    for (int slot = 0; slot < 4; slot++) {
-        const int c = slot * 32 + lane;
-        if (c < nchunks) {
-            float v[8];
-#pragma unroll
-            for (int l = 0; l < 8; l++) { v[l] = ggml_v_expf_dev(__fsub_rn(p[c * 8 + l], mx)); }
-#pragma unroll
-            for (int l = 0; l < 8; l++) p[c * 8 + l] = v[l];
-            const float t0 = __fadd_rn(v[4], v[0]), t1 = __fadd_rn(v[5], v[1]), t2 = __fadd_rn(v[6], v[2]), t3 = __fadd_rn(v[7], v[3]);
-            csum[slot] = __fadd_rn(__fadd_rn(t0, t2), __fadd_rn(t1, t3));
-        }
-    }
-    for (int i = nchunks * 8; i < n_kv; i++) {
-        const float val = glibc_expf_dev(__fsub_rn(p[i], mx));
-        if (lane == 0) p[i] = val;
-    }
-    __syncwarp();
-    double tsum = 0.0;
-#pragma unroll
-    for (int slot = 0; slot < 4; slot++) tsum += (double) csum[slot];
-#pragma unroll
-    for (int o = 16; o > 0; o >>= 1) tsum += __shfl_xor_sync(0xffffffffu, tsum, o);
-    float sc;
-    {
-        const double dl = 2.0 * (double)(nchunks + 8) * 0x1p-53 * tsum * (1.0 + 1e-6);
-        double lo = tsum - dl, hi = tsum + dl;
-        for (int i = nchunks * 8; i < n_kv; i++) { const double tl = (double) p[i]; lo = __dadd_rn(lo, tl); hi = __dadd_rn(hi, tl); }
-        const double mid = 0.5 * (lo + hi);
-        double y = (double) __frcp_rn((float) mid);
-        double e = __fma_rn(-mid, y, 1.0); y = __fma_rn(y, e, y);
-        e = __fma_rn(-mid, y, 1.0);        y = __fma_rn(y, e, y);
-        const double rw = (hi - lo) * y * 0.5 + 0x1p-48;
-        sc = __double2float_rn(y * (1.0 - rw));
-        if (sc != __double2float_rn(y * (1.0 + rw))) {
-            double sum = 0.0;
-#pragma unroll
-            for (int slot = 0; slot < 4; slot++) {
-                const int base = slot * 32;
-                if (base < nchunks) {
-                    const int cnt = min(32, nchunks - base);
-                    for (int l = 0; l < cnt; l++) sum = __dadd_rn(sum, (double) __shfl_sync(0xffffffffu, csum[slot], l));
-                }
-            }
-            for (int i = nchunks * 8; i < n_kv; i++) sum = __dadd_rn(sum, (double) p[i]);
-            sc = __double2float_rn(__ddiv_rn(1.0, sum));
-        }
-    }
-    __syncwarp();
-    for (int i = lane; i < n_kv; i += 32) p[i] = __fmul_rn(p[i], sc);
-}
-
-__global__ void attn_softmax_kernel(float * __restrict__ S, int rows, int n_kv) {
-    const int row = blockIdx.x * (blockDim.x >> 5) + (threadIdx.x >> 5);
-    if (row >= rows) return;
-    softmax_row(S + (size_t) row * n_kv, n_kv);
-}
-
-__global__ void attn_pv_kernel(const float * __restrict__ S, const float * __restrict__ Vc, int N, int n_kv, int E, int H, int D,
-                               void * __restrict__ act, int wt, int Kp) {
-    const int d = threadIdx.x, q = blockIdx.x * blockDim.y + threadIdx.y, h = blockIdx.y;
-    if (q >= N || d >= D) return;
-    const float * p = S + ((size_t) h * N + q) * n_kv;
-    const float * v = Vc + h * D + d;
-    float acc[32];
-#pragma unroll
-    for (int l = 0; l < 32; l++) acc[l] = 0.0f;
-    const int np = n_kv & ~31;
-    for (int k0 = 0; k0 < np; k0 += 32) {
-#pragma unroll
-        for (int l = 0; l < 32; l++) acc[l] = __fmaf_rn(v[(size_t)(k0 + l) * E], p[k0 + l], acc[l]);
-    }
-    store_act(act, wt, Kp, q, h * D + d, pv_leftovers(lane_tree_reduce_local(acc), v, p, np, n_kv, E));
 }
 
 __device__ __forceinline__ float * row_cache(float * const (&p)[8], int b) {
@@ -411,31 +304,4 @@
     BARK_LAUNCH(attn_pv_batch_kernel, dim3(D / 8, H, B), 32, 0, s, scores, kv, d_pos, E, D, max_kv, act, (int) wt, Kp);
 }
 
-void attention(const float * Q, const float * Kc, const float * Vc, int N, int n_kv, int n_past, int E, int H, bool causal,
-               float * scores, void * act, WType wt, int Kp, cudaStream_t s) {
-    const int D = E / H;
-    const float scale = 1.0f / sqrtf((float) E / (float) H);
-    const int rows = H * N;
-    if (use_tiled() && D % 32 == 0 && D <= 128) {
-        g_next_bytes = 4.0 * ((double) n_kv * E + (double) N * E + (double) H * N * n_kv); g_next_flops = 2.0 * (double) N * n_kv * E;
-        attention_tiled_scores(Q, Kc, N, n_kv, n_past, E, H, scale, causal, scores, s);
-        g_next_bytes = 8.0 * (double) rows * n_kv;
-        BARK_LAUNCH(attn_softmax_kernel, (rows + 7) / 8, 256, 0, s, scores, rows, n_kv);
-        g_next_bytes = 4.0 * ((double) n_kv * E + (double) H * N * n_kv + (double) N * E); g_next_flops = 2.0 * (double) N * n_kv * E;
-        attention_tiled_pv(scores, Vc, N, n_kv, E, H, act, wt, Kp, s);
-        return;
-    }
-    g_next_bytes = 4.0 * ((double) n_kv * E + (double) N * E + (double) H * N * n_kv); g_next_flops = 2.0 * (double) N * n_kv * E;
-    if (D == 64)       BARK_LAUNCH(attn_scores_kernel<2>, (rows + 7) / 8, 256, 0, s, Q, Kc, N, n_kv, n_past, E, H, scale, causal ? 1 : 0, scores);
-    else if (D == 32)  BARK_LAUNCH(attn_scores_kernel<1>, (rows + 7) / 8, 256, 0, s, Q, Kc, N, n_kv, n_past, E, H, scale, causal ? 1 : 0, scores);
-    else if (D == 96)  BARK_LAUNCH(attn_scores_kernel<3>, (rows + 7) / 8, 256, 0, s, Q, Kc, N, n_kv, n_past, E, H, scale, causal ? 1 : 0, scores);
-    else if (D == 128) BARK_LAUNCH(attn_scores_kernel<4>, (rows + 7) / 8, 256, 0, s, Q, Kc, N, n_kv, n_past, E, H, scale, causal ? 1 : 0, scores);
-    else { fprintf(stderr, "bark_b200: unsupported head size %d (need a multiple of 32, <= 128)\n", D); throw std::runtime_error("unsupported configuration (see the message above)"); }
-    g_next_bytes = 8.0 * (double) rows * n_kv;
-    BARK_LAUNCH(attn_softmax_kernel, (rows + 7) / 8, 256, 0, s, scores, rows, n_kv);
-    const int qy = max(1, 256 / D);
-    g_next_bytes = 4.0 * ((double) n_kv * E + (double) H * N * n_kv + (double) N * E); g_next_flops = 2.0 * (double) N * n_kv * E;
-    BARK_LAUNCH(attn_pv_kernel, dim3((N + qy - 1) / qy, H), dim3(D, qy), 0, s, scores, Vc, N, n_kv, E, H, D, act, (int) wt, Kp);
-}
-
-}
+}
diff --git a/bark.cpp_b200/csrc/gpt_kernels.h b/bark.cpp_b200/csrc/gpt_kernels.h
--- a/bark.cpp_b200/csrc/gpt_kernels.h
+++ b/bark.cpp_b200/csrc/gpt_kernels.h
@@ -25,8 +25,10 @@
 
 void lane_matmul(const DMat & W, const void * act, int act_gs, int rows, const MatmulEpilogue & ep, cudaStream_t s);
 
+enum AttnPath : int { ATTN_AUTO = 0, ATTN_FUSED = 1, ATTN_TILED = 2 };
+int  attn_tiled_max_rows(int H, int n_sm);
 void attention(const float * Q, const float * Kc, const float * Vc, int N, int n_kv, int n_past, int E, int H, bool causal,
-               float * scores, void * act, WType wt, int Kp, cudaStream_t s);
+               float * scores, void * act, WType wt, int Kp, cudaStream_t s, AttnPath path = ATTN_AUTO);
 
 struct BatchKV { float * k[8], * v[8]; };
 void attention_batch(const float * Q, const float * Kst, const float * Vst, const BatchKV & kv, const int32_t * d_pos, int B, int max_kv, int E, int H,
@@ -45,8 +47,6 @@
 void   qx_matmul(const DMat & W, const void * act_f32, int ld_act, int rows, const MatmulEpilogue & ep, cudaStream_t s);
 
 void lane_gemm_tiled(const DMat & W, const void * act, int act_gs, int rows, const MatmulEpilogue & ep, cudaStream_t s);
-void attention_tiled_scores(const float * Q, const float * Kc, int N, int n_kv, int n_past, int E, int H, float scale, bool causal, float * scores, cudaStream_t s);
-void attention_tiled_pv(const float * scores, const float * Vc, int N, int n_kv, int E, int H, void * act, WType wt, int Kp, cudaStream_t s);
 
 enum { FEPI_F32 = 0, FEPI_RESID = 1, FEPI_GELU16 = 2, FEPI_QKV16 = 4 };
 struct FastEpi {
diff --git a/include/bark_b200.h b/include/bark_b200.h
--- a/include/bark_b200.h
+++ b/include/bark_b200.h
@@ -48,6 +48,9 @@
 BARK_API int  bark_b200_fast_gemm(const uint16_t * A, const uint16_t * W, void * C, int M, int N, int K, int epilogue, int bn);
 BARK_API int  bark_b200_fast_attention(const uint16_t * q, const uint16_t * k, const uint16_t * v, uint16_t * out, int n, int E, int H);
 
+BARK_API int  bark_b200_parity_attention(const float * q, const float * k, const float * v, float * out, int N, int n_kv, int n_past, int E, int H, int causal,
+                                         int path);
+
 #ifdef __cplusplus
 }
 #endif
```

Result: faster. 12.14, median of 6 (+5.8%).
